# UT-Austin-RPL/FORGE

Hardware: AMD Instinct MI355X
Metric: rendered views/sec (5 views, 128^2 px, 64^3 voxel) (higher is better)
Workload: dtype f32; 1 GPU; BASELINE configs[1]: FORGE hot path, 1 scene(s)/GPU x 5 input views 256^2 -> 32^3x128 feature grid -> 64^3 render grid -> 5 views x 128^2 rays x 64 samples -> 5 RGB 256^2; HIP rotate, fp32-MFMA implicit-GEMM ResNet-50 trunk / conv1 / ConvGRU (Winograd F(2x2,3x3) x 3 depth taps) / heads / conv_rgb, HIP ray-march (no MIOpen/rocBLAS kernel in the step); eval BN, random-init seeded weights; scenes_per_gpu=1, views_in=5, views_out=5, feature_grid=32, render_grid=64, steps_in_flight=4, launch=hipGraph replay, 4 steps in flight on 4 HIP streams, parallelism=dp1 (scene-sharded, no data-path collective; 4-scalar RCC...

## Files before the change

forge_amd/_lib.py:

```python
import ctypes
import os

import torch

_HERE = os.path.dirname(os.path.abspath(__file__))
LIB_PATH = os.environ.get("FORGE_AMD_LIB") or os.path.join(_HERE, "libforge_hip.so")
_lib = None

_P = ctypes.c_void_p
_I = ctypes.c_int
_F = ctypes.c_float
_D = ctypes.c_double
_LL = ctypes.c_longlong

SIGNATURES = {
    "forge_version": [],
    "forge_last_error": [],
    "forge_rotate_fwd": [_P, _P, _P, _P, _I, _I, _I, _I, _I, _P],
    "forge_rotate_fwd_slots": [_P, _P, _P, _P, _P, _I, _I, _I, _I, _I, _P],
    "forge_rotate_xf_from_poses": [_P, _P, _P, _P, _P, _I, _I, _F, _P],
    "forge_rotate_bwd": [_P, _P, _P, _P, _P, _P, _I, _I, _I, _I, _I, _P],
    "forge_pose_chain_fwd": [_P, _P, _P, _P, _P, _F, _I, _I, _P, _P, _P, _P, _P, _P, _P, _P],
    "forge_colsum": [_P, _I, _P, _P, _LL, _I, _P],
    "forge_adam_small": [_P, _P, _P, _P, _P, _I, _F, _F, _F, _F, _P],
    "forge_rotate_bwd_slots": [_P, _P, _P, _P, _P, _P, _P, _I, _I, _I, _I, _I, _P],
    "forge_pose_chain_bwd": [_P, _P, _P, _P, _P, _I, _I, _P],
    "forge_pack_cameras": [_P, _LL, _LL, _LL, _P, _LL, _LL, _P, _LL, _LL, _LL, _P, _P, _I, _P],
    "forge_render_fwd": [_P, _P, _P, _P, _P, _P, _P] + [_I] * 9 + [_F] * 5 + [_P],
    "forge_render_bwd_ws_bytes": [_I] * 6,
    "forge_render_bwd": [_P, _P, _P, _P, _P, _P, _P, _P, _P, _P] + [_I] * 9 + [_F] * 5 + [_P, _LL, _P],
    "forge_resize_bilinear_fwd": [_P, _P, _I, _I, _I, _I, _I, _P],
    "forge_resize_bilinear_bwd": [_P, _P, _I, _I, _I, _I, _I, _P],
    "forge_conv_igemm": [_P, _I, _I, _LL, _P, _I, _I, _LL, _P, _P, _P, _P, _F, _P, _P, _P, _P, _P, _P] + [_I] * 10 + [_P] + [_I] * 12 + [_P, _LL, _P, _P],
    "forge_wino_weights": [_P, _P, _I, _I, _I, _I, _P],
    "forge_wino_dy": [_P, _I, _P, _I, _I, _I, _I, _I, _P],
    "forge_wino_wgrad": [_P, _P, _I, _LL, _LL, _P, _I, _LL, _LL, _P, _I, _I, _I, _I, _I, _I, _P],
    "forge_wino_dw": [_P, _P, _I, _I, _I, _P],
    "forge_wino_input": [_P, _I, _LL, _P, _I, _LL, _I, _I, _I, _I, _I, _I, _LL, _P],
    "forge_wino_input_dy": [_P, _I, _P, _P, _I, _I, _I, _I, _I, _P],
    "forge_wino_gemm": [_P, _I, _I, _LL, _LL, _P, _I, _I, _LL, _LL, _P, _P, _I, _I, _I, _I, _I, _I, _I, _P],
    "forge_wino_gemm_half": [_P, _I, _I, _LL, _LL, _P, _I, _I, _LL, _LL, _P, _P, _I, _I, _I, _I, _I, _I, _P],
    "forge_wino_gemm_dn": [_P, _I, _I, _LL, _LL, _P, _I, _I, _LL, _LL, _P, _P, _I, _I, _I, _I, _I, _I, _P],
    "forge_wino_weights_dn": [_P, _P, _I, _I, _P],
    "forge_wino_input_dn4": [_P, _I, _LL, _P, _I, _LL, _I, _I, _I, _I, _I, _I, _LL, _P],
    "forge_wino_weights_dn4": [_P, _P, _I, _I, _P],
    "forge_wino_gemm_dn4": [_P, _I, _I, _LL, _LL, _P, _I, _I, _LL, _LL, _P, _P, _I, _I, _I, _I, _I, _I, _P],
    "forge_wino_output_half": [_P, _P, _LL, _LL, _P, _P, _P, _F, _P, _P, _P, _P, _P, _P, _I, _I, _I, _I, _I, _I, _I, _P],
    "forge_wino_gemm_tile": [_LL, _I, _I],
    "forge_wino_output": [_P, _P, _LL, _LL, _P, _P, _P, _F, _P, _P, _P, _P, _P, _P, _I, _I, _I, _I, _I, _I, _I, _P],
    "forge_conv_igemm_plan": [_LL, _I, _I, _I, _I, _I, _I, _LL, _P, _P],
    "forge_conv_wgrad": [_P, _I, _P, _I, _I, _LL, _P, _I, _I, _LL, _P] + [_I] * 9 + [_P, _I, _P],
    "forge_conv_direct_fwd": [_P, _I, _P, _P, _F, _P, _I] + [_I] * 6 + [_P, _I, _P],
    "forge_conv_direct_dgrad": [_P, _I, _P, _P, _I] + [_I] * 6 + [_P, _I, _P],
    "forge_conv_direct_wgrad": [_P, _I, _P, _I, _P] + [_I] * 6 + [_P, _I, _P],
    "forge_gru_gates_fwd": [_P, _P, _P, _P, _P, _LL, _I, _P],
    "forge_gru_state_fwd": [_P, _P, _P, _P, _LL, _I, _P],
    "forge_gru_state_bwd": [_P, _I, _P, _P, _P, _P, _P, _P, _LL, _I, _P, _LL, _LL, _I, _P],
    "forge_gru_gates_bwd": [_P, _P, _I, _P, _P, _P, _P, _P, _P, _I, _LL, _I, _P, _LL, _LL, _I, _P],
    "forge_bn_ws_doubles": [_I],
    "forge_bn_train_fwd": [_P, _I, _P, _P, _F, _F, _P, _I, _P, _P, _P, _P, _F, _P, _LL, _I, _P, _I, _P, _I, _P],
    "forge_bn_train_bwd": [_P, _I, _P, _I, _P, _P, _P, _P, _F, _P, _I, _P, _P, _P, _LL, _I, _P, _I, _P, _I, _P],
    "forge_bn_sync_stats": [_P, _I, _P, _LL, _I, _I, _P],
    "forge_bn_eval_fwd": [_P, _I, _P, _P, _P, _P, _F, _F, _P, _I, _P, _P, _LL, _I, _P, _I, _P],
    "forge_bn_sync_fwd_apply": [_P, _I, _P, _P, _F, _F, _P, _I, _P, _P, _P, _P, _F, _P, _LL, _LL, _I, _P, _I, _P, _P],
    "forge_bn_sync_bwd_reduce": [_P, _I, _P, _I, _P, _P, _P, _P, _F, _P, _P, _P, _LL, _I, _P, _I, _P],
    "forge_bn_sync_bwd_apply": [_P, _I, _P, _I, _P, _P, _P, _P, _F, _P, _I, _P, _LL, _LL, _I, _P, _I, _P, _I, _P],
    "forge_affine_act_bwd": [_P, _I, _P, _I, _P, _F, _P, _I, _LL, _I, _P],
    "forge_sse_groups_blocks": [],
    "forge_sse_groups_fwd": [_P, _LL, _LL, _LL, _LL, _P, _P] + [_I] * 7 + [_P],
    "forge_sse_groups_bwd": [_P, _LL, _LL, _LL, _LL, _P, _P, _P] + [_I] * 7 + [_P],
    "forge_attention_fwd": [_P, _P, _P, _LL, _P, _I, _I, _I, _I, _P],
    "forge_attention_fwd_lse": [_P, _P, _P, _LL, _P, _P, _I, _I, _I, _I, _P],
    "forge_attention_bwd": [_P, _P, _P, _LL, _P, _P, _P, _P, _P, _P, _P, _I, _I, _I, _I, _P],
    "forge_attention_mh_fwd": [_P, _P, _P, _P, _P, _I, _I, _I, _I, _I] + [_LL] * 8 + [_F, _P],
    "forge_attention_mh_bwd": [_P] * 10 + [_I, _I, _I, _I, _I] + [_LL] * 8 + [_F, _P],
    "forge_token_linear_fwd": [_P, _LL, _P, _P, _P, _P, _F, _P, _LL, _P, _LL, _P, _P, _I, _I, _I, _I, _P],
    "forge_layer_norm_fwd": [_P, _LL, _P, _P, _F, _P, _LL, _P, _I, _I, _P],
    "forge_token_rows_plan": [_I, _I, _I, _P, _P],
    "forge_token_linear_bwd_ws_bytes": [_I, _I, _I, _I],
    "forge_token_linear_bwd": [_P, _LL, _P, _LL] + [_P] * 11 + [_LL, _I, _I, _I, _I, _P],
    "forge_layer_norm_bwd_ws_bytes": [_I, _I],
    "forge_layer_norm_bwd": [_P, _LL, _P, _LL] + [_P] * 6 + [_LL, _I, _I, _P],
    "forge_im2col_nchw": [_P, _P] + [_I] * 9 + [_P],
    "forge_maxpool2d_nhwc": [_P, _P] + [_I] * 7 + [_P],
    "forge_vgg_prep_fwd": [_P, _LL, _LL, _LL, _LL, _P, _LL, _LL, _LL, _LL, _P, _P, _P] + [_I] * 7 + [_P],
    "forge_vgg_prep_bwd": [_P, _I, _P, _P, _LL, _LL, _LL, _LL] + [_I] * 7 + [_P],
    "forge_l1_partial_blocks": [],
    "forge_l1_partial": [_P, _P, _LL, _P, _P],
    "forge_vgg_tap_bwd": [_P, _P, _P, _P, _P, _I, _I, _I, _I, _P],
    "forge_conv_wgrad_det": [_P, _I, _P, _I, _I, _LL, _P, _I, _I, _LL, _P] + [_I] * 9 + [_P, _I, _I, _P, _LL, _P],
    "forge_conv_wgrad_det_ws_bytes": [_I] * 11 + [_P, _I],
    "forge_conv_wgrad_plan": [_I] * 11 + [_P, _I, _I, _P],
    "forge_wino_wgrad_det": [_P, _P, _I, _LL, _LL, _P, _I, _LL, _LL, _P, _I, _I, _I, _I, _I, _I, _I, _P, _LL, _P],
    "forge_wino_wgrad_det_ws_bytes": [_I] * 8,
    "forge_conv_direct_wgrad_det": [_P, _I, _P, _I, _P] + [_I] * 6 + [_P, _I, _I, _P, _LL, _P],
    "forge_conv_direct_wgrad_det_ws_bytes": [_I] * 7,
    "forge_rotate_bwd_det": [_P, _P, _P, _P, _P, _P, _I, _I, _I, _I, _I, _I, _P, _LL, _P],
    "forge_rotate_bwd_det_ws_bytes": [_I] * 5,
    "forge_rotate_bwd_slots_det": [_P, _P, _P, _P, _P, _P, _P, _I, _I, _I, _I, _I, _I, _P, _LL, _P],
    "forge_rotate_bwd_slots_det_ws_bytes": [_I] * 5,
    "forge_metric_blocks": [],
    "forge_ssim_tiles": [_I, _I],
    "forge_psnr": [_P, _LL, _LL, _LL, _LL, _P, _LL, _LL, _LL, _LL, _I, _I, _I, _I, _D, _P, _P, _P],
    "forge_ssim": [_P, _LL, _LL, _LL, _LL, _P, _LL, _LL, _LL, _LL, _I, _I, _I, _I, _D, _P, _P, _P],
    "forge_lpips_tap": [_P, _I, _I, _I, _P, _P, _P],
    "forge_lpips_finalize": [_P, _I, _I, _I, _I, _I, _I, _P, _P],
    "forge_pose_sync": [_P, _P, _P, _I, _I, _I, _I, _I, _D, _P, _P, _P, _P],
    "forge_mesh_case_table": [_P, _I],
    "forge_mesh_workspace_bytes": [_I, _I, _I, _I],
    "forge_mesh_count": [_P, _I, _I, _I, _I, _F, _P, _LL, _P, _P],
    "forge_mesh_emit": [_P, _P, _I, _I, _I, _I, _I, _F, _F, _P, _LL, _P, _P, _I, _I, _P, _P, _P, _P, _P, _P],
    "forge_ncdhw_to_ndhwc": [_P, _P, _I, _I, _LL, _P],
    "forge_ndhwc_to_ncdhw": [_P, _P, _I, _I, _LL, _P],
}


_LL_RESULTS = ("forge_render_bwd_ws_bytes", "forge_conv_wgrad_det_ws_bytes", "forge_wino_wgrad_det_ws_bytes",
               "forge_conv_direct_wgrad_det_ws_bytes", "forge_rotate_bwd_det_ws_bytes", "forge_rotate_bwd_slots_det_ws_bytes",
               "forge_token_linear_bwd_ws_bytes", "forge_layer_norm_bwd_ws_bytes", "forge_mesh_workspace_bytes")


def lib():
    global _lib
    if _lib is None:
        if not os.path.exists(LIB_PATH):
            raise RuntimeError(
                "forge_amd: %s not found. Build it with `python -m forge_amd.build` (needs hipcc, "
                "targets gfx950). There is no CPU/PyTorch fallback for the HIP kernels." % LIB_PATH)
        h = ctypes.CDLL(LIB_PATH)
# ... 36 lines not shown
```

forge_amd/convops.py:

```python
import collections
import ctypes
import functools
import os
from fractions import Fraction

import torch

from . import _lib, determinism

EPI_BIAS, EPI_AFFINE_ACT, EPI_GRU_GATES, EPI_GRU_OUT = 0, 1, 2, 3


_TAPS_CACHE = {}


def _taps_array(taps):
    key = tuple(tuple(t) for t in taps)
    arr = _TAPS_CACHE.get(key)
    if arr is None:
        flat = [int(v) for t in key for v in t]
        arr = _TAPS_CACHE[key] = (ctypes.c_int * len(flat))(*flat)
    return arr


# ... 93 lines not shown
        return super().train(mode)

    def _apply(self, fn, *args, **kwargs):
        self.invalidate_packed()
        return super()._apply(fn, *args, **kwargs)


def invalidate_packed(module):
    for m in module.modules():
        if isinstance(m, PackedModule):
            m.invalidate_packed()


class _ZeroArena:

    def __init__(self):
        self.task, self.device = -1, None
        self.pools = {}
        self.want = {}

    def _end(self):
        self.want = {k: p[2] for k, p in self.pools.items()}
        self.pools, self.task = {}, -1

    HAVE_HOOKS = hasattr(torch._C, "_current_graph_task_id") and hasattr(getattr(torch.autograd.Variable, "_execution_engine", None), "queue_callback")

    def zeros(self, shape, device):
        n = 1
        for d in shape:
            n *= int(d)
        nbytes = (n * 4 + 255) // 256 * 256
        if not self.HAVE_HOOKS:
            return torch.zeros(shape, dtype=torch.float32, device=device)
        task = torch._C._current_graph_task_id()
        if task < 0:
            return torch.zeros(shape, dtype=torch.float32, device=device)
        if task != self.task:
            if self.task >= 0:
                self._end()
            self.task, self.device = task, device
            torch.autograd.Variable._execution_engine.queue_callback(self._end_of(task))
        if device != self.device:
            return torch.zeros(shape, dtype=torch.float32, device=device)
        key = torch.cuda.current_stream(device).cuda_stream if torch.device(device).type == "cuda" else 0
        pool = self.pools.get(key)
        if pool is None:
            want = self.want.get(key, 0)
            pool = self.pools[key] = [torch.zeros(want // 4 + 64, dtype=torch.float32, device=device) if want else None, 0, 0]
        pool[2] += nbytes
        if pool[0] is None or pool[1] + nbytes > pool[0].numel() * 4:
            return torch.zeros(shape, dtype=torch.float32, device=device)
        out = pool[0][pool[1] // 4:pool[1] // 4 + n].view(shape)
        pool[1] += nbytes
        return out

    def _end_of(self, task):
        def cb():
            if self.task == task:
                self._end()
        return cb


GRAD_ZEROS = _ZeroArena()


def grad_zeros(shape, device, scratch=False):
    if scratch:
        return torch.zeros(tuple(shape), dtype=torch.float32, device=device)
    return GRAD_ZEROS.zeros(tuple(shape), device)


SPLITK_WS_BYTES = 128 << 20

TILE_NAMES = {"A": "128, 128, 8, 1", "B": "64, 128, 8, 1", "C": "128, 64, 8, 1", "D": "64, 64, 4, 1", "E": "128, 32, 4, 1"}

_PLAN_CACHE = {}


class _State:
    plan_override = None
    winograd = True
    wino_depth_nest = os.environ.get("FORGE_WINO_DEPTH_NEST", "1") != "0"
    wino_depth_nest4 = os.environ.get("FORGE_WINO_DEPTH_NEST4", "1") != "0"


STATE = _State()


class force_plan:

    def __init__(self, tile=None, ksplit=None):
        self.val = (tile, ksplit)

    def __enter__(self):
        self.prev = STATE.plan_override
        STATE.plan_override = self.val
        return self

    def __exit__(self, *exc):
        STATE.plan_override = self.prev
        return False


def conv_plan(M, Cout, Cin, ntaps, epilogue, ldo, nphase=1):
    key = (int(M), int(Cout), int(Cin), int(ntaps), int(nphase), int(epilogue), int(ldo) % 4 == 0)
    pl = _PLAN_CACHE.get(key)
    if pl is None:
        tile, ks = ctypes.c_int(0), ctypes.c_int(0)
        _lib.check(_lib.lib().forge_conv_igemm_plan(int(M), int(Cout), int(Cin), int(ntaps), int(nphase), int(epilogue), int(ldo), SPLITK_WS_BYTES,
                                                    ctypes.byref(tile), ctypes.byref(ks)), "forge_conv_igemm_plan")
        pl = _PLAN_CACHE[key] = (chr(tile.value), ks.value)
    ov = STATE.plan_override
    if ov is not None and pl[0] != "N":
        tile = ov[0] or pl[0]
        ks = ov[1] if ov[1] is not None else (pl[1] if ov[0] is None else 1)
        can_split = nphase == 1 and epilogue in (EPI_BIAS, EPI_AFFINE_ACT) and Cout % 4 == 0 and ldo % 4 == 0
        if ks > 1 and not (can_split and ks * M * Cout * 4 <= SPLITK_WS_BYTES and ks <= (ntaps // nphase) * (Cin // 32)):
            ks = 1
        return tile, ks
    return pl


MAX_OPERAND_BYTES = (1 << 31) - 1


@_lib.on_tensor_device
def conv_igemm(in1, C1, ld1, in2, C2, ld2, wp, bias, scale, shift, slope, residual, aux_h, aux_z, out, out2,
               grid, in_grid, Cout, ldo, taps, out_grid=None, istride=1, ostride=1, phase=(0, 0, 0), epilogue=EPI_BIAS,
               bs1=0, bs2=0, lift=0, out3=None, stats=None):
    n, D, H, W = grid
    Di, Hi, Wi = in_grid
    Do, Ho, Wo = out_grid if out_grid is not None else (D, H, W)
    if wp.shape != (len(taps), Cout, C1 + C2):
        raise ValueError("packed weight %s does not match taps=%d Cout=%d Cin=%d" % (tuple(wp.shape), len(taps), Cout, C1 + C2))
    in_rows, out_rows = Di * Hi * Wi, Do * Ho * Wo
    b1, b2 = (int(bs1) or in_rows), (int(bs2) or in_rows)
    span = lambda k, br, ld: ((k - 1) * br + in_rows) * ld * 4
    limit = MAX_OPERAND_BYTES
    nc = n
    while nc > 1 and (span(nc, b1, ld1) > limit or (in2 is not None and span(nc, b2, ld2) > limit)):
        nc = (nc + 1) // 2
    L, st, arr = _lib.lib(), _lib.current_stream(), _taps_array(taps)
    nphase = 1
    if tuple(phase) == (-1, -1, -1):
        nphase = 8 if Do == 2 * D else 4

    def off(t, floats):
        return None if t is None else ctypes.c_void_p(t.data_ptr() + 4 * floats)
    gate_w = Cout // 2 if epilogue == EPI_GRU_GATES else Cout
    for s0 in range(0, n, nc):
        k = min(nc, n - s0)
        orow = s0 * out_rows
        tile, ksplit = conv_plan(k * D * H * W, Cout, C1 + C2, len(taps), epilogue, ldo, nphase)
        if stats is not None and (ksplit > 1 or nc < n):
            raise RuntimeError("forge_amd: conv_igemm output statistics need an un-chunked launch without split-K (use conv_stats_buffer)")
        ws = torch.empty(ksplit * k * D * H * W * Cout, dtype=torch.float32, device=out.device) if ksplit > 1 else None
        o_ld = gate_w if epilogue == EPI_GRU_GATES else ldo
        _lib.check(L.forge_conv_igemm(
            off(in1, s0 * b1 * ld1), C1, ld1, int(bs1), off(in2, s0 * b2 * ld2), C2, ld2, int(bs2), _lib.ptr(wp), _lib.ptr(bias), _lib.ptr(scale),
            _lib.ptr(shift), float(slope), off(residual, orow * (Cout if (lift or epilogue in (EPI_GRU_GATES, EPI_GRU_OUT)) else ldo)),
            off(aux_h, orow * gate_w), off(aux_z, orow * Cout),
            off(out, orow * (Cout if lift else o_ld)), off(out2, orow * o_ld), off(out3, orow * o_ld), k, D, H, W, istride, Di, Hi, Wi, Cout, ldo,
            arr, len(taps), ostride, phase[0], phase[1], phase[2], Do, Ho, Wo, epilogue, int(lift), 0 if tile == "N" else ord(tile), ksplit,
            _lib.ptr(ws), 0 if ws is None else ws.numel() * 4, _lib.ptr(stats), st),
            "forge_conv_igemm")
    return out
# ... 56 lines not shown
    return v


def conv3_launch(x1, C1, x2, C2, wp, bias, out, grid, Cout, bs1=0, residual=None, dgrad=False, U=None, wT=None):
    n, D, H, W = grid
    if wino_applies(TAPS_3x3x3, 1, n, D, H, W, C1, C2, Cout):
        return _wino_conv(x1, C1, bs1, x2, C2, 0, U if U is not None else wino_pack_packed(wp, transpose=dgrad), bias, out, residual, grid)
    w = (wT if wT is not None else wp.transpose(1, 2).contiguous()) if dgrad else wp
    taps = [(-a, -b, -c) for a, b, c in TAPS_3x3x3] if dgrad else TAPS_3x3x3
    if residual is None:
        return conv_igemm(x1, C1, C1, x2, C2, C2, w, bias, None, None, 1.0, None, None, None, out, None, grid, (D, H, W), Cout, Cout, taps,
                          epilogue=EPI_BIAS, bs1=bs1)
    one, zero = _one_zero(out.device, Cout)
    return conv_igemm(x1, C1, C1, x2, C2, C2, w, bias, one, zero, 1.0, residual, None, None, out, None, grid, (D, H, W), Cout, Cout, taps,
                      epilogue=EPI_AFFINE_ACT, bs1=bs1)


def wino_wgrad_applies(n, D, H, W, C1, C2, Cout, taps=None):
    return (wino_applies(TAPS_3x3x3 if taps is None else taps, 1, n, D, H, W, C1, C2, Cout) and C1 + C2 >= 128 and Cout >= 64 and (C2 == 0 or C1 % 128 == 0)
            and n * D * (H // 2) * (W // 2) * Cout * 4 <= MAX_OPERAND_BYTES)


@_lib.on_tensor_device
def conv3_wgrad(dy, x1, C1, x2, C2, dwp, grid, Cout, bs1=0, taps=None, dM=None):
    n, D, H, W = grid
    taps = TAPS_3x3x3 if taps is None else list(taps)
    if not wino_wgrad_applies(n, D, H, W, C1, C2, Cout, taps):
        return conv_wgrad(dy, x1, C1, x2, C2, dwp, grid, (D, H, W), Cout, taps, bs1=bs1)
    kd = len(taps) // 9
    L, st = _lib.lib(), _lib.current_stream()
    Ht, Wt = H // 2, W // 2
    R = n * D * Ht * Wt
    dev = dy.device
    V1 = wino_input(x1, C1, C1, n, D, H, W, bs=bs1)
    V2 = None if x2 is None else wino_input(x2, C2, C2, n, D, H, W)
    if dM is None:
        dM = torch.empty(16, R, Cout, dtype=torch.float32, device=dev)
        _lib.check(L.forge_wino_dy(_lib.ptr(dy), dy.shape[-1], _lib.ptr(dM), n, D, H, W, Cout, st), "forge_wino_dy")
    dU = grad_zeros((16, kd, Cout, C1 + C2), dev, scratch=True)
    determinism.launch("forge_wino_wgrad", (_lib.ptr(dM), _lib.ptr(V1), C1, 0, 0, _lib.ptr(V2), C2, 0, 0, _lib.ptr(dU), n, D, Ht, Wt, Cout, kd),
                       (C1, C2, n, D, Ht, Wt, Cout, kd), dev)
    _lib.check(L.forge_wino_dw(_lib.ptr(dU), _lib.ptr(dwp), Cout, C1 + C2, kd, st), "forge_wino_dw")
    return dwp


def wino_applies(taps, istride, n, D, H, W, C1, C2, Cout):
    tt = tuple(tuple(t) for t in taps)
    if not (wino_enabled() and istride == 1 and C1 % 32 == 0 and C2 % 32 == 0 and Cout % 8 == 0 and wino_fits(n, D, H, W, max(C1, C2, 1))):
        return False
    if len(tt) == 27 and tt == tuple(TAPS_3x3x3):
        return C1 + C2 >= 64 and Cout >= 32
    if len(tt) == 9 and tt == tuple(TAPS_3x3) and D == 1:
        return C2 == 0 and C1 >= WINO2D_MIN_C and Cout >= WINO2D_MIN_C
    return False


def wino_enabled():
    return STATE.winograd


class winograd:

    def __init__(self, on):
        self.on = bool(on)

    def __enter__(self):
        self.prev = STATE.winograd
        STATE.winograd = self.on
        return self

    def __exit__(self, *exc):
        STATE.winograd = self.prev
        return False


def wino_scene_chunk(b, D, H, W, C, views=1):
    nb = b
    while nb >= 1 and not wino_fits(nb, D, H, W, C, views=views):
        nb = (nb + 1) // 2 if nb > 1 else 0
    return nb


def wino_fits(n, D, H, W, C, views=1, nest4=False, form=None):
    rows = n * views * D * (H // 2) * (W // 2) * (form or WINO_FORMS["dn4" if nest4 else "points"]).rows
    return H % 2 == 0 and W % 2 == 0 and rows * C * 4 <= MAX_OPERAND_BYTES


@_lib.on_tensor_device
def wino_input_dy(dy, C, n, D, H, W):
    R = n * D * (H // 2) * (W // 2)
    V = torch.empty(16, R, C, dtype=torch.float32, device=dy.device)
    dM = torch.empty(16, R, C, dtype=torch.float32, device=dy.device)
    _lib.check(_lib.lib().forge_wino_input_dy(_lib.ptr(dy), C, _lib.ptr(V), _lib.ptr(dM), n, D, H, W, C, _lib.current_stream()), "forge_wino_input_dy")
    return V, dM


def wino_half_applies(R, Cout, Cin):
    return STATE.plan_override is None and wino_gemm_tile(R, Cout, Cin) == "B"


def wino_depth_nest_applies(R, D, Ht, Wt, Cout, Cin):
    return (STATE.wino_depth_nest and STATE.plan_override is None and D % 2 == 0 and (Ht * Wt) % 64 == 0 and Cin % 32 == 0
            and R * Cout * 4 <= MAX_OPERAND_BYTES and wino_gemm_tile(R, Cout, Cin) == "B")


def wino_depth_nest4_applies(R, D, Ht, Wt, Cout, Cin):
    return STATE.wino_depth_nest4 and D % 4 == 0 and D >= 8 and wino_depth_nest_applies(R, D, Ht, Wt, Cout, Cin)


WinoForm = collections.namedtuple("WinoForm", "name P gemm weights ushape input rows kloops applies tile metered")
_U4 = lambda kd, co_, ci_: (16, kd, co_, ci_)
WINO_FORMS = {f.name: f for f in (
    WinoForm("points", 16, "forge_wino_gemm", "forge_wino_weights", _U4, "forge_wino_input", 1, None, lambda R, D, Ht, Wt, Cout, Cin: True,
             True, True),
    WinoForm("half", 8, "forge_wino_gemm_half", "forge_wino_weights", _U4, "forge_wino_input", 1, None,
             lambda R, D, Ht, Wt, Cout, Cin: wino_half_applies(R, Cout, Cin), False, True),
    WinoForm("dn", 16, "forge_wino_gemm_dn", "forge_wino_weights_dn", lambda kd, co_, ci_: (16, 2, 2, co_, ci_), "forge_wino_input", 1, 2,
             lambda *a: wino_depth_nest_applies(*a), False, True),
    WinoForm("dn4", 16, "forge_wino_gemm_dn4", "forge_wino_weights_dn4", lambda kd, co_, ci_: (16, 6, co_, ci_), "forge_wino_input_dn4", Fraction(3, 2),
             Fraction(3, 2), lambda *a: wino_depth_nest4_applies(*a), False, False),
)}


def wino_calls(form):
    if not form.metered:
        return functools.partial(wino_form_input, form), functools.partial(wino_form_gemm, form)
    return (lambda *a, **kw: wino_input(*a, **kw)), (lambda *a, **kw: wino_gemm(*a, **kw))


@_lib.on_tensor_device
def wino_pack(form, wp, transpose=False):
    T, co_, ci_ = wp.shape
    nest = form.kloops is not None
    assert T == 27 or (T == 9 and not nest)
    assert not (nest and transpose)
    kd = T // 9
    wp = wp.detach()
    wp = wp if wp.is_contiguous() else wp.contiguous()
    U = torch.empty(form.ushape(kd, ci_, co_) if transpose else form.ushape(kd, co_, ci_), dtype=torch.float32, device=wp.device)
    own = () if nest else (kd, 1 if transpose else 0)
    _lib.check(getattr(_lib.lib(), form.weights)(_lib.ptr(wp), _lib.ptr(U), co_, ci_, *own, _lib.current_stream()), form.weights)
    return U


@_lib.on_tensor_device
def wino_form_input(form, x, C, ld, n, D, H, W, bs=0, out=None, nsum=1, sum_stride=0):
    rows = int(n * D * (H // 2) * (W // 2) * form.rows)
    V = out if out is not None else torch.empty(16, rows, C, dtype=torch.float32, device=x.device)
    if form.rows != 1 and (V.shape != (16, rows, C) or not V.is_contiguous()):
        raise ValueError("depth-nest operand buffer %s is not [16][%d][%d]" % (tuple(V.shape), rows, C))
    _lib.check(getattr(_lib.lib(), form.input)(_lib.ptr(x), ld, int(bs), _lib.ptr(V), C, 0, n, D, H, W, C, int(nsum), int(sum_stride), _lib.current_stream()),
               form.input)
    return V


def wino_input(x, C, ld, n, D, H, W, bs=0, out=None, nsum=1, sum_stride=0):
    return wino_form_input(WINO_FORMS["points"], x, C, ld, n, D, H, W, bs=bs, out=out, nsum=nsum, sum_stride=sum_stride)


def _point_products(Mm, P, R, Cout, device):
    if Mm is None:
        Mm = torch.empty(P, R, Cout, dtype=torch.float32, device=device)
    if not (Mm.is_contiguous() and Mm.dtype == torch.float32 and Mm.numel() >= P * R * Cout):
        raise ValueError("point-product buffer %s %s%s cannot hold %d x %d x %d float32" % (
            tuple(Mm.shape), Mm.dtype, "" if Mm.is_contiguous() else " (not contiguous)", P, R, Cout))
    if Mm.shape != (P, R, Cout):
        Mm = Mm.as_strided((P, R, Cout), (R * Cout, Cout, 1))
    return Mm


@_lib.on_tensor_device
def wino_form_gemm(form, V1, C1, V2, C2, U, Mm, n, D, Ht, Wt, Cout, view=0, views=1):
    R = n * D * Ht * Wt
    vol = int(D * Ht * Wt * form.rows)
    nest = form.kloops is not None
    kd = 3 if nest else U.shape[1]
    if U.shape != form.ushape(kd, Cout, C1 + C2) or (kd not in (1, 3)) or (nest and not U.is_contiguous()):
        raise ValueError("%s weight %s does not match Cout=%d Cin=%d" % ("depth-nest" if nest else "transformed", tuple(U.shape), Cout, C1 + C2))
    if form.rows != 1 and (V1.shape[1] != n * views * vol or (V2 is not None and V2.shape[1] != n * vol)):
        raise ValueError("depth-nest operands %s / %s are not %s's %d (x %d views) rows per point" % (
            tuple(V1.shape), None if V2 is None else tuple(V2.shape), form.input, n * vol, views))
    Mm = _point_products(Mm, form.P, R, Cout, V1.device)
    tile = (ord(wino_gemm_tile(R, Cout, C1 + C2)),) if form.tile else ()
    p1 = ctypes.c_void_p(V1.data_ptr() + 4 * view * vol * C1)
    _lib.check(getattr(_lib.lib(), form.gemm)(p1, C1, C1, views * vol if views > 1 else 0, V1.shape[1] * C1, _lib.ptr(V2), C2, C2, 0,
                                              0 if V2 is None else V2.shape[1] * C2, _lib.ptr(U), _lib.ptr(Mm), n, D, Ht, Wt, Cout, kd,
                                              *tile, _lib.current_stream()), form.gemm)
    return Mm


def wino_gemm(V1, C1, V2, C2, U, Mm, n, D, Ht, Wt, Cout, view=0, views=1, half=None):
    if U.dim() == 5:
        form = "dn"
    else:
        if half is None:
            half = WINO_FORMS["half"].applies(n * D * Ht * Wt, D, Ht, Wt, Cout, C1 + C2)
        form = "half" if half else "points"
    return wino_form_gemm(WINO_FORMS[form], V1, C1, V2, C2, U, Mm, n, D, Ht, Wt, Cout, view=view, views=views)


def wino_gemm_tile(R, Cout, Cin):
    ov = STATE.plan_override
    if ov is not None and ov[0]:
        return ov[0]
    return chr(_lib.lib().forge_wino_gemm_tile(int(R), int(Cout), int(Cin)))


@_lib.on_tensor_device
def wino_output(Mm, bias, scale, shift, slope, residual, aux_h, aux_z, out, out2, out3, n, D, H, W, Cout, ldo, epilogue, Mm2=None, view=0, views=1):
    vol = D * (H // 2) * (W // 2)
    P = Mm.shape[0] if Mm.dim() == 3 else 0
    if P not in (8, 16) or Mm.shape[1:] != (n * vol, Cout) or not Mm.is_contiguous():
        raise ValueError("point products %s do not match [8 | 16][%d][%d]" % (tuple(Mm.shape), n * vol, Cout))
    if Mm2 is not None and (Mm2.shape != (P, n * views * vol, Cout) or not Mm2.is_contiguous()):
        raise ValueError("second addend %s does not match [%d][%d][%d] (the form of Mm)" % (tuple(Mm2.shape), P, n * views * vol, Cout))
    p2 = None if Mm2 is None else ctypes.c_void_p(Mm2.data_ptr() + 4 * view * vol * Cout)
    fn, name = (_lib.lib().forge_wino_output_half, "forge_wino_output_half") if P == 8 else (_lib.lib().forge_wino_output, "forge_wino_output")
    _lib.check(fn(_lib.ptr(Mm), p2, views * vol, 0 if Mm2 is None else Mm2.shape[1] * Cout, _lib.ptr(bias), _lib.ptr(scale), _lib.ptr(shift), float(slope),
                  _lib.ptr(residual), _lib.ptr(aux_h), _lib.ptr(aux_z), _lib.ptr(out), _lib.ptr(out2), _lib.ptr(out3), n, D, H, W, Cout, ldo, epilogue,
                  _lib.current_stream()), name)
    return out


@_lib.on_tensor_device
def conv_wgrad(dy, x1, C1, x2, C2, dwp, grid, in_grid, Cout, taps, istride=1, bs1=0, bs2=0):
    if x2 is not None and C1 % 128:
        x1 = torch.cat([x1[..., :C1], x2[..., :C2]], dim=-1)
        C1, x2, C2, bs1, bs2 = C1 + C2, None, 0, 0, 0
    n, D, H, W = grid
    Di, Hi, Wi = in_grid
    in_rows, out_rows = Di * Hi * Wi, D * H * W
    ldy, ld1, ld2 = dy.shape[-1], x1.shape[-1], (0 if x2 is None else x2.shape[-1])
    b1, b2 = (int(bs1) or in_rows), (int(bs2) or in_rows)
    span = lambda k, br, ld, rows: ((k - 1) * br + rows) * ld * 4
    nc = n
    while nc > 1 and (span(nc, out_rows, ldy, out_rows) > MAX_OPERAND_BYTES or span(nc, b1, ld1, in_rows) > MAX_OPERAND_BYTES
                      or (x2 is not None and span(nc, b2, ld2, in_rows) > MAX_OPERAND_BYTES)):
        nc = (nc + 1) // 2
    off = lambda t, floats: None if t is None else ctypes.c_void_p(t.data_ptr() + 4 * floats)
    ta = _taps_array(taps)
    for s0 in range(0, n, nc):
        k = min(nc, n - s0)
        determinism.launch("forge_conv_wgrad", (off(dy, s0 * out_rows * ldy), ldy, off(x1, s0 * b1 * ld1), C1, ld1, int(bs1), off(x2, s0 * b2 * ld2), C2, ld2,
                                                int(bs2), _lib.ptr(dwp), k, D, H, W, istride, Di, Hi, Wi, Cout, ta, len(taps)),
                           (C1, C2, k, D, H, W, istride, Di, Hi, Wi, Cout, ta, len(taps)), dwp.device)
    return dwp


def _batch_stride_rows(x):
    n, D, H, W, C = x.shape
    if x.stride()[1:] != (H * W * C, W * C, C, 1):
        raise ValueError("conv_rows needs channels-last rows [n,D,H,W,C] dense within a batch element; got strides %s" % (x.stride(),))
    return 0 if (n == 1 or x.stride(0) == D * H * W * C) else x.stride(0) // C


@_lib.on_tensor_device
def colsum(x):
    C = x.shape[-1]
    rows = x.reshape(-1, C)
    if not (rows.is_cuda and rows.dtype == torch.float32):
        raise RuntimeError("forge_amd: colsum runs only on the MI355X HIP kernels (float32 cuda tensor); got %s on %s" % (rows.dtype, rows.device))
    if C % 4:
        if C > 32:
            raise RuntimeError("forge_amd: colsum needs C %% 4 == 0 or C <= 32 (got %d)" % C)
        rows = rows if rows.is_contiguous() else rows.contiguous()
    else:
        rows = rows if (rows.stride(1) == 1 and rows.stride(0) >= C and rows.stride(0) % 4 == 0) else rows.contiguous()
    out = torch.empty(C, dtype=torch.float32, device=rows.device)
    ws = torch.empty(_lib.lib().forge_bn_ws_doubles(C), dtype=torch.float64, device=rows.device)
    _lib.check(_lib.lib().forge_colsum(_lib.ptr(rows), rows.stride(0), _lib.ptr(out), _lib.ptr(ws), rows.shape[0], C, _lib.current_stream()), "forge_colsum")
    return out


class _ConvTapsRows(torch.autograd.Function):

    @staticmethod
    def forward(ctx, x1, x2, wp, bias, taps, istride, out_spatial, want_stats=False):
        n, Di, Hi, Wi, C1 = x1.shape
        C2 = 0 if x2 is None else x2.shape[-1]
        T, Cout, Cin = wp.shape
        D, H, W = out_spatial
        wpc = wp.detach().contiguous()
        out = torch.empty(n, D, H, W, Cout, dtype=torch.float32, device=x1.device)
        bs1 = _batch_stride_rows(x1)
        bs2 = 0 if x2 is None else _batch_stride_rows(x2)
        stats = None
        if (D, H, W) == (Di, Hi, Wi) and wino_applies(taps, istride, n, D, H, W, C1, C2, Cout):
            wino_conv_rows(x1, x2, wino_pack_packed(wpc), bias, out)
        else:
            if want_stats and bs1 == 0 and bs2 == 0:
                stats = conv_stats_buffer(x1, x2, (n, D, H, W), (Di, Hi, Wi), Cout, Cin, T, Cout, x1.device)
            conv_igemm(x1, C1, C1, x2, C2, C2, wpc, bias, None, None, 1.0, None, None, None, out, None,
                       (n, D, H, W), (Di, Hi, Wi), Cout, Cout, taps, istride=istride, epilogue=EPI_BIAS, bs1=bs1, bs2=bs2, stats=stats)
        ctx.save_for_backward(x1, x2, wpc)
        ctx.meta = (tuple(taps), istride, (D, H, W), bias is not None)
        if not want_stats:
# ... 308 lines not shown
```

forge_amd/csrc/conv_igemm.hip:

```cpp
#include "common.h"
#include <cmath>
#include <type_traits>

namespace forge {

enum ConvEpilogue : int {
    EPI_BIAS = 0,
    EPI_AFFINE_ACT = 1,
    EPI_GRU_GATES = 2,
    EPI_GRU_OUT = 3,
};

constexpr int MAX_TAPS = 64;

struct ConvArgs {
    const float* in1; const float* in2;
    int C1, C2, ld1, ld2;
    long long bs1r, bs2r;
    long long span1, span2;
    const float* wp;
    const float* bias;
    const float* scale; const float* shift; float slope;
    const float* aux_h; const float* aux_z;
    float* out; float* out2; float* out3;
// ... 1033 lines not shown
                  "forge_conv_igemm: row strides must cover the channels and keep 16-byte alignment");
    ConvArgs a;
    a.in1 = in1; a.in2 = in2; a.C1 = C1; a.C2 = C2; a.ld1 = ld1; a.ld2 = ld2;
    a.bs1r = bs1 > 0 ? bs1 : (long long)Di * Hi * Wi; a.bs2r = bs2 > 0 ? bs2 : (long long)Di * Hi * Wi;
    a.span1 = ((long long)(n - 1) * a.bs1r + (long long)Di * Hi * Wi) * ld1 * 4;
    a.span2 = in2 ? ((long long)(n - 1) * a.bs2r + (long long)Di * Hi * Wi) * ld2 * 4 : 0;
    FORGE_REQUIRE(a.span1 < (1ll << 31) && a.span2 < (1ll << 31) && (long long)ntaps * Cout * (C1 + C2) * 4 < (1ll << 31), FORGE_ESHAPE,
                  "forge_conv_igemm: an operand spans >= 2 GiB (32-bit buffer offsets); split the batch");
    a.is = is; a.Di = Di; a.Hi = Hi; a.Wi = Wi; a.residual = residual;
    a.ldr = (lift > 0 || epilogue == EPI_GRU_GATES || epilogue == EPI_GRU_OUT) ? Cout : ldo;
    a.lift = lift; a.ws = nullptr; a.ksplit = 1; a.stats = stats;
    a.wp = wp; a.bias = bias; a.scale = scale; a.shift = shift; a.slope = slope;
    a.aux_h = aux_h; a.aux_z = aux_z; a.out = out; a.out2 = out2; a.out3 = out3; a.n = n; a.D = D; a.H = H; a.W = W; a.Cout = Cout; a.ldo = ldo;
    a.ntaps = ntaps; a.os = os; a.pz = pz; a.py = py; a.px = px; a.Do = Do; a.Ho = Ho; a.Wo = Wo; a.epi = epilogue;
    a.nphase = 1; a.tpp = ntaps; a.nbat = 1; a.pt1 = a.pt2 = a.ptw = a.pto = 0;
    if (pz < 0) {
        FORGE_REQUIRE(os == 2 && py < 0 && px < 0 && Ho == 2 * H && Wo == 2 * W && (Do == 2 * D || Do == D), FORGE_EINVAL,
                      "forge_conv_igemm: merged phases (pz = py = px = -1) need os = 2 and a doubled output grid");
        a.nphase = Do == 2 * D ? 8 : 4;
        FORGE_REQUIRE(ntaps % a.nphase == 0, FORGE_EINVAL, "forge_conv_igemm: merged phases need ntaps %% %d == 0", a.nphase);
        a.tpp = ntaps / a.nphase;
        a.pz = a.py = a.px = 0;
    }
    for (int k = 0; k < 3 * ntaps; ++k)
        FORGE_REQUIRE(taps[k] >= -128 && taps[k] <= 127, FORGE_EINVAL, "forge_conv_igemm: tap %d component %d = %d outside [-128, 127]", k / 3, k % 3, taps[k]);
    for (int t = 0; t < MAX_TAPS; ++t) {
        for (int k = 0; k < 3; ++k) a.tap[t][k] = (signed char)(t < ntaps ? taps[t * 3 + k] : 0);
        a.tap[t][3] = 0;
    }
    const long long M = (long long)n * D * H * W;
    FORGE_REQUIRE(M < (1ll << 31), FORGE_ESHAPE, "forge_conv_igemm: more than 2^31 GEMM rows; split the batch");
    FORGE_REQUIRE(out3 == nullptr || epilogue == EPI_GRU_GATES || epilogue == EPI_GRU_OUT, FORGE_EINVAL, "forge_conv_igemm: out3 is a GRU-epilogue output");
    hipStream_t st = (hipStream_t)stream;
    if (Cout <= 16) {
        FORGE_REQUIRE(epilogue == EPI_BIAS || epilogue == EPI_AFFINE_ACT, FORGE_EINVAL, "forge_conv_igemm: GRU epilogues need Cout > 16");
        const long long grid = (M + BM16 - 1) / BM16 * a.nphase;
        FORGE_REQUIRE(grid < (1ll << 31), FORGE_ESHAPE, "forge_conv_igemm: grid too large");
        int lines_r = 0;
        if (a.nphase == 1 && is == 1 && os == 1 && lift == 0 && Do == D && Ho == H && Wo == W && Di == D && Hi == H && Wi == W && pz == 0 && py == 0 && px == 0) {
            for (int r = 1; r <= 2 && !lines_r; ++r) {
                const int nt = 2 * r + 1;
                bool ok = ntaps % nt == 0 && W > r;
                for (int t = 0; ok && t < ntaps; ++t)
                    ok = taps[t * 3 + 2] == (t % nt) - r && taps[t * 3] == taps[(t - t % nt) * 3] && taps[t * 3 + 1] == taps[(t - t % nt) * 3 + 1];
                if (ok) lines_r = r;
            }
        }
        if (lines_r == 1) hipLaunchKernelGGL(conv_igemm_n16_lines_kernel<1>, dim3((unsigned)grid), dim3(NTHREADS), 0, st, a);
        else if (lines_r == 2) hipLaunchKernelGGL(conv_igemm_n16_lines_kernel<2>, dim3((unsigned)grid), dim3(NTHREADS), 0, st, a);
        else hipLaunchKernelGGL(conv_igemm_n16_kernel, dim3((unsigned)grid), dim3(NTHREADS), 0, st, a);
    } else {
        const bool can_split = a.nphase == 1 && splitk_ws && (epilogue == EPI_BIAS || epilogue == EPI_AFFINE_ACT) && Cout % 4 == 0 && ldo % 4 == 0;
        ConvPlan pl;
        if (tile == 0) {
            pl = plan_conv(M * a.nphase, Cout, C1 + C2, a.tpp, can_split, splitk_ws_bytes);
        } else {
            pl = ConvPlan{(char)tile, ksplit > 1 ? ksplit : 1};
            FORGE_REQUIRE(tile >= 'A' && tile <= 'E', FORGE_EINVAL, "forge_conv_igemm: tile '%c' is not one of A..E (0 = planned here)", (char)tile);
            FORGE_REQUIRE(pl.ksplit == 1 || (can_split && pl.ksplit <= 8 && (long long)pl.ksplit * M * Cout * 4 <= splitk_ws_bytes &&
                                             pl.ksplit <= a.tpp * ((C1 + C2) / BK)), FORGE_EINVAL,
                          "forge_conv_igemm: ksplit=%d needs epilogue 0/1 without phases, Cout, ldo %% 4 == 0 and a workspace of ksplit M Cout floats", pl.ksplit);
        }
        FORGE_REQUIRE(stats == nullptr || (tile != 0 && pl.ksplit == 1), FORGE_EINVAL,
                      "forge_conv_igemm: output statistics need an explicit tile ('A'..'E' from forge_conv_igemm_plan) and a plan without split-K");
        if (pl.ksplit > 1) { a.ksplit = pl.ksplit; a.ws = splitk_ws; }
        if (int rc = launch_conv_tile(a, pl.tile, st)) return rc;
        if (a.ksplit > 1) {
            const long long total = M * (Cout / 4);
            hipLaunchKernelGGL(conv_splitk_epilogue_kernel, dim3((unsigned)((total + 255) / 256)), dim3(256), 0, st, a);
        }
    }
    FORGE_LAUNCH_CHECK("forge_conv_igemm");
    return 0;
}

extern "C" int forge_wino_gemm_tile(long long R, int Cout, int Cin) {
    (void)Cin;
    if (Cout <= 64) return R < 2048 ? 'D' : 'C';
    return R < 2048 ? 'D' : 'B';
}

static int wino_gemm_impl(const float* V1, int C1, int ld1, long long bs1, long long pt1, const float* V2, int C2, int ld2, long long bs2,
                          long long pt2, const float* U, float* Mm, int n, int D, int Ht, int Wt, int Cout, int kd, int tile, int form, forge_stream_t stream) {
    const bool half = form == 1, dn = form == 2, dn4 = form == 3;
    FORGE_REQUIRE(tile == 0 || (tile >= 'A' && tile <= 'E'), FORGE_EINVAL, "forge_wino_gemm: tile must be 0 (default rule) or 'A'..'E'");
    FORGE_REQUIRE(V1 && U && Mm && (kd == 1 || kd == 3), FORGE_EINVAL, "forge_wino_gemm: null pointer argument / kd not 1 or 3");
    FORGE_REQUIRE(n > 0 && D > 0 && Ht > 0 && Wt > 0 && Cout > 16, FORGE_EINVAL, "forge_wino_gemm: bad dims n=%d D=%d Ht=%d Wt=%d Cout=%d (Cout > 16)", n,
                  D, Ht, Wt, Cout);
    FORGE_REQUIRE(C1 > 0 && C1 % BK == 0 && C2 >= 0 && C2 % BK == 0 && (C2 == 0) == (V2 == nullptr), FORGE_ESHAPE,
                  "forge_wino_gemm: C1=%d / C2=%d must be multiples of %d, V2 given iff C2 > 0", C1, C2, BK);
    FORGE_REQUIRE(ld1 >= C1 && ld1 % 4 == 0 && (C2 == 0 || (ld2 >= C2 && ld2 % 4 == 0)), FORGE_EINVAL, "forge_wino_gemm: bad row strides");
    FORGE_REQUIRE(!dn || (kd == 3 && D % 2 == 0 && ((long long)Ht * Wt) % 64 == 0), FORGE_EINVAL,
                  "forge_wino_gemm_dn: needs three depth taps, an even D and Ht Wt %% 64 == 0 (kd=%d D=%d Ht=%d Wt=%d)", kd, D, Ht, Wt);
    FORGE_REQUIRE(!dn4 || (kd == 3 && D % 4 == 0 && ((long long)Ht * Wt) % 64 == 0), FORGE_EINVAL,
                  "forge_wino_gemm_dn4: needs three depth taps, D %% 4 == 0 and Ht Wt %% 64 == 0 (kd=%d D=%d Ht=%d Wt=%d)", kd, D, Ht, Wt);
    ConvArgs a;
    memset(&a, 0, sizeof(a));
    const long long vol = (long long)D * Ht * Wt, R = (long long)n * vol, rows = dn4 ? vol / 4 * 6 : vol, Cin = C1 + C2;
    const int npos = dn4 ? 6 : dn ? 4 : kd;
    a.in1 = V1; a.in2 = V2; a.C1 = C1; a.C2 = C2; a.ld1 = ld1; a.ld2 = ld2; a.bs1r = bs1 > 0 ? bs1 : rows; a.bs2r = bs2 > 0 ? bs2 : rows;
    a.span1 = ((long long)(n - 1) * a.bs1r + rows) * ld1 * 4;
    a.span2 = V2 ? ((long long)(n - 1) * a.bs2r + rows) * ld2 * 4 : 0;
    if (dn4) {
        FORGE_REQUIRE(a.span1 < (1ll << 31) && a.span2 < (1ll << 31) && R * Cout * 4 < (1ll << 31) && 6ll * Cout * Cin * 4 < (1ll << 31), FORGE_EINVAL,
                      "forge_wino_gemm_dn4: an operand or an output plane spans >= 2 GiB (32-bit buffer offsets); split the batch");
    } else {
        FORGE_REQUIRE(a.span1 < (1ll << 31) && a.span2 < (1ll << 31) && R < (1ll << 31), FORGE_ESHAPE,
                      "forge_wino_gemm: an operand spans >= 2 GiB per Winograd point (32-bit buffer offsets); split the batch");
        FORGE_REQUIRE(!dn || (R * Cout * 4 < (1ll << 31) && 4ll * Cout * Cin * 4 < (1ll << 31)), FORGE_ESHAPE,
                      "forge_wino_gemm_dn: an output plane spans >= 2 GiB (32-bit buffer offsets); split the batch");
    }
    a.wp = U; a.slope = 1.f; a.out = Mm; a.n = n; a.D = D; a.H = Ht; a.W = Wt; a.is = 1; a.Di = D; a.Hi = Ht; a.Wi = Wt;
    a.Cout = Cout; a.ldo = Cout; a.ldr = Cout; a.ntaps = a.tpp = npos; a.os = 1; a.Do = D; a.Ho = Ht; a.Wo = Wt; a.nphase = 1; a.epi = EPI_BIAS;
    a.ksplit = 1; a.nbat = half ? 4 : 16;
    a.pt1 = pt1 > 0 ? pt1 : (long long)n * rows * ld1; a.pt2 = V2 ? (pt2 > 0 ? pt2 : (long long)n * rows * ld2) : 0;
    a.ptw = (long long)npos * Cout * Cin; a.pto = R * Cout;
    if (form == 0 || half) {
        if (kd == 3) { a.tap[0][0] = -1; a.tap[2][0] = 1; }
        if (!tile) tile = forge_wino_gemm_tile(R, Cout, C1 + C2);
    }
    if (int rc = launch_conv_tile(a, (char)tile, (hipStream_t)stream, form)) return rc;
    FORGE_LAUNCH_CHECK(dn4 ? "forge_wino_gemm_dn4" : dn ? "forge_wino_gemm_dn" : "forge_wino_gemm");
    return 0;
}

extern "C" int forge_wino_gemm(const float* V1, int C1, int ld1, long long bs1, long long pt1, const float* V2, int C2, int ld2, long long bs2,
                               long long pt2, const float* U, float* Mm, int n, int D, int Ht, int Wt, int Cout, int kd, int tile, forge_stream_t stream) {
    return wino_gemm_impl(V1, C1, ld1, bs1, pt1, V2, C2, ld2, bs2, pt2, U, Mm, n, D, Ht, Wt, Cout, kd, tile, 0, stream);
}

extern "C" int forge_wino_gemm_half(const float* V1, int C1, int ld1, long long bs1, long long pt1, const float* V2, int C2, int ld2, long long bs2,
                                    long long pt2, const float* U, float* Mm8, int n, int D, int Ht, int Wt, int Cout, int kd, forge_stream_t stream) {
    return wino_gemm_impl(V1, C1, ld1, bs1, pt1, V2, C2, ld2, bs2, pt2, U, Mm8, n, D, Ht, Wt, Cout, kd, 'B', 1, stream);
}

extern "C" int forge_wino_gemm_dn(const float* V1, int C1, int ld1, long long bs1, long long pt1, const float* V2, int C2, int ld2, long long bs2,
                                  long long pt2, const float* Ud, float* Mm, int n, int D, int Ht, int Wt, int Cout, int kd, forge_stream_t stream) {
    FORGE_REQUIRE(C1 > 0 && C1 % BK == 0 && C2 >= 0 && C2 % BK == 0, FORGE_EINVAL, "forge_wino_gemm_dn: C1=%d / C2=%d must be multiples of %d", C1, C2, BK);
    return wino_gemm_impl(V1, C1, ld1, bs1, pt1, V2, C2, ld2, bs2, pt2, Ud, Mm, n, D, Ht, Wt, Cout, kd, 'B', 2, stream);
}

extern "C" int forge_wino_gemm_dn4(const float* V1, int C1, int ld1, long long bs1, long long pt1, const float* V2, int C2, int ld2, long long bs2,
                                   long long pt2, const float* Ud, float* Mm, int n, int D, int Ht, int Wt, int Cout, int kd, forge_stream_t stream) {
    FORGE_REQUIRE(C1 > 0 && C1 % BK == 0 && C2 >= 0 && C2 % BK == 0, FORGE_EINVAL, "forge_wino_gemm_dn4: C1=%d / C2=%d must be multiples of %d", C1, C2, BK);
    return wino_gemm_impl(V1, C1, ld1, bs1, pt1, V2, C2, ld2, bs2, pt2, Ud, Mm, n, D, Ht, Wt, Cout, kd, 'B', 3, stream);
}
```

forge_amd/csrc/winograd.hip:

```cpp
#include "common.h"

namespace forge {

__device__ __forceinline__ float4 add(float4 a, float4 b) { return make_float4(a.x + b.x, a.y + b.y, a.z + b.z, a.w + b.w); }
__device__ __forceinline__ float4 sub(float4 a, float4 b) { return make_float4(a.x - b.x, a.y - b.y, a.z - b.z, a.w - b.w); }
__device__ __forceinline__ float add(float a, float b) { return a + b; }
__device__ __forceinline__ float sub(float a, float b) { return a - b; }

__device__ __forceinline__ void tile_decode(long long idx, int per, int cs, int Ht, int Wt, unsigned& r, int& c, int& tw, int& th, unsigned& t) {
    r = (unsigned)(idx / per);
    c = (int)(idx - (long long)r * per) << cs;
    unsigned q = r;
    t = q / (unsigned)Wt;
    tw = (int)(q - t * (unsigned)Wt); q = t; t = q / (unsigned)Ht;
    th = (int)(q - t * (unsigned)Ht);
}

template <typename T, typename I>
__device__ __forceinline__ void bt_d_b_store(const T (&d)[4][4], float* V, I row, int ld, int c, long long ptv) {
    T w[4][4];
#pragma unroll
    for (int j = 0; j < 4; ++j) {
        w[0][j] = sub(d[0][j], d[2][j]);
        w[1][j] = add(d[1][j], d[2][j]);
        w[2][j] = sub(d[2][j], d[1][j]);
        w[3][j] = sub(d[1][j], d[3][j]);
    }
    float* vp = V + (long long)row * ld + c;
#pragma unroll
    for (int i = 0; i < 4; ++i) {
        *reinterpret_cast<T*>(vp + (4 * i + 0) * ptv) = sub(w[i][0], w[i][2]);
        *reinterpret_cast<T*>(vp + (4 * i + 1) * ptv) = add(w[i][1], w[i][2]);
        *reinterpret_cast<T*>(vp + (4 * i + 2) * ptv) = sub(w[i][2], w[i][1]);
        *reinterpret_cast<T*>(vp + (4 * i + 3) * ptv) = sub(w[i][1], w[i][3]);
    }
}

__device__ __forceinline__ void a_y_at_store(float4 y00, float4 y01, float4 y10, float4 y11, float* mp, long long ptm) {
    const float4 zero = make_float4(0.f, 0.f, 0.f, 0.f);
    const float4 s[4][2] = {{y00, y01}, {add(y00, y10), add(y01, y11)}, {sub(y00, y10), sub(y01, y11)}, {sub(zero, y10), sub(zero, y11)}};
#pragma unroll
    for (int i = 0; i < 4; ++i) {
        *reinterpret_cast<float4*>(mp + (4 * i + 0) * ptm) = s[i][0];
        *reinterpret_cast<float4*>(mp + (4 * i + 1) * ptm) = add(s[i][0], s[i][1]);
        *reinterpret_cast<float4*>(mp + (4 * i + 2) * ptm) = sub(s[i][0], s[i][1]);
        *reinterpret_cast<float4*>(mp + (4 * i + 3) * ptm) = sub(zero, s[i][1]);
    }
}

__device__ __forceinline__ void g_d_gt_store(const double (&d)[3][3], float* up, long long pt) {
    double g[4][3];
#pragma unroll
    for (int b = 0; b < 3; ++b) {
        g[0][b] = d[0][b];
        g[1][b] = 0.5 * (d[0][b] + d[1][b] + d[2][b]);
        g[2][b] = 0.5 * (d[0][b] - d[1][b] + d[2][b]);
        g[3][b] = d[2][b];
    }
#pragma unroll
    for (int i = 0; i < 4; ++i) {
        up[(4 * i + 0) * pt] = (float)g[i][0];
        up[(4 * i + 1) * pt] = (float)(0.5 * (g[i][0] + g[i][1] + g[i][2]));
        up[(4 * i + 2) * pt] = (float)(0.5 * (g[i][0] - g[i][1] + g[i][2]));
        up[(4 * i + 3) * pt] = (float)g[i][2];
    }
}

struct WinoInArgs {
    const float* in; int ld; long long bs;
    float* V; int ldv; long long ptv;
    int n, D, H, W, C;
    int nsum; long long ss;
    float* dM; long long ptm;
};

template <bool DY>
__global__ __launch_bounds__(256) void wino_input_kernel(const WinoInArgs a) {
    const int C4 = a.C >> 2, Ht = a.H >> 1, Wt = a.W >> 1;
    const long long idx = (long long)xcd_remap(blockIdx.x, gridDim.x) * 256 + threadIdx.x;
    const long long R = (long long)a.n * a.D * Ht * Wt;
    if (idx >= R * C4) return;
    unsigned r, t;
    int c, tw, th;
    tile_decode(idx, C4, 2, Ht, Wt, r, c, tw, th, t);
    const unsigned q = t; t = q / (unsigned)a.D;
    const int z = (int)(q - t * (unsigned)a.D);
    const float* base = a.in + ((long long)t * a.bs + (long long)z * a.H * a.W) * a.ld + c;
    float4 d[4][4];
#pragma unroll
    for (int i = 0; i < 4; ++i) {
        const int y = 2 * th - 1 + i;
#pragma unroll
        for (int j = 0; j < 4; ++j) {
            const int x = 2 * tw - 1 + j;
            const bool ok = (unsigned)y < (unsigned)a.H && (unsigned)x < (unsigned)a.W;
            float4 v = make_float4(0.f, 0.f, 0.f, 0.f);
            if (ok) {
                const float* p = base + ((long long)y * a.W + x) * a.ld;
                v = *reinterpret_cast<const float4*>(p);
                if (a.nsum > 1) {
                    for (int k = 1; k < a.nsum; ++k) v = add(v, *reinterpret_cast<const float4*>(p + (long long)k * a.ss * a.ld));
                    const float inv = 1.f / (float)a.nsum;
                    v = make_float4(v.x * inv, v.y * inv, v.z * inv, v.w * inv);
                }
            }
            d[i][j] = v;
        }
    }
    if constexpr (DY) a_y_at_store(d[1][1], d[1][2], d[2][1], d[2][2], a.dM + (long long)r * a.C + c, a.ptm);
    bt_d_b_store(d, a.V, r, a.ldv, c, a.ptv);
}

__global__ __launch_bounds__(256) void wino_input_dn4_kernel(const WinoInArgs a) {
    const int Ht = a.H >> 1, Wt = a.W >> 1, Dg = a.D >> 2;
    const long long idx = (long long)xcd_remap(blockIdx.x, gridDim.x) * 256 + threadIdx.x;
    const long long RG = (long long)a.n * Dg * Ht * Wt;
    if (idx >= RG * a.C) return;
    unsigned r, t;
    int c, tw, th;
    tile_decode(idx, a.C, 0, Ht, Wt, r, c, tw, th, t);
    const unsigned q = t; t = q / (unsigned)Dg;
    const int g = (int)(q - t * (unsigned)Dg);
    const long long HW = (long long)a.H * a.W;
    const float* base = a.in + (long long)t * a.bs * a.ld + c;
    const float inv = 1.f / (float)a.nsum;
    float d[6][4][4];
#pragma unroll
    for (int i = 0; i < 4; ++i) {
        const int y = 2 * th - 1 + i;
#pragma unroll
        for (int j = 0; j < 4; ++j) {
            const int x = 2 * tw - 1 + j;
            const bool ok = (unsigned)y < (unsigned)a.H && (unsigned)x < (unsigned)a.W;
            float p[6];
#pragma unroll
            for (int e = 0; e < 6; ++e) {
                const int z = 4 * g - 1 + e;
                float v = 0.f;
                if (ok && (unsigned)z < (unsigned)a.D) {
                    const float* s = base + ((long long)z * HW + (long long)y * a.W + x) * a.ld;
                    v = *s;
                    if (a.nsum > 1) {
                        for (int k = 1; k < a.nsum; ++k) v += s[(long long)k * a.ss * a.ld];
                        v *= inv;
                    }
                }
                p[e] = v;
            }
            const float a02 = p[0] - p[2], a24 = p[2] - p[4], s34 = p[3] + p[4], s12 = p[1] + p[2], d43 = p[4] - p[3], d12 = p[1] - p[2];
            const float d42 = p[4] - p[2], d31 = p[3] - p[1], d13 = p[1] - p[3], d35 = p[3] - p[5];
            d[0][i][j] = fmaf(4.f, a02, -a24);
            d[1][i][j] = fmaf(-4.f, s12, s34);
            d[2][i][j] = fmaf(4.f, d12, d43);
            d[3][i][j] = fmaf(2.f, d31, d42);
            d[4][i][j] = fmaf(-2.f, d31, d42);
            d[5][i][j] = fmaf(4.f, d13, -d35);
        }
    }
    const long long HWt = (long long)Ht * Wt;
    float* vp = a.V + ((((long long)t * Dg + g) * 6) * HWt + (long long)th * Wt + tw) * a.ldv + c;
#pragma unroll
    for (int k = 0; k < 6; ++k) bt_d_b_store(d[k], vp, k * HWt, a.ldv, 0, a.ptv);
}

__global__ __launch_bounds__(256) void wino_weight_kernel(const float* __restrict__ wp, float* __restrict__ U, int Cout, int Cin, int KD, int transpose) {
    const int No = transpose ? Cin : Cout, Nc = transpose ? Cout : Cin;
    const long long idx = (long long)blockIdx.x * 256 + threadIdx.x, per = (long long)No * Nc;
    if (idx >= KD * per) return;
    const int kd = (int)(idx / per);
    const long long oc = idx - kd * per;
    const int o = (int)(oc / Nc), c = (int)(oc - (long long)o * Nc);
    double w[3][3];
#pragma unroll
    for (int a = 0; a < 3; ++a)
#pragma unroll
        for (int b = 0; b < 3; ++b) {
            const int tap = transpose ? ((KD - 1 - kd) * 3 + (2 - a)) * 3 + (2 - b) : (kd * 3 + a) * 3 + b;
            w[a][b] = (double)wp[((long long)tap * Cout + (transpose ? c : o)) * Cin + (transpose ? o : c)];
        }
    g_d_gt_store(w, U + ((long long)kd * No + o) * Nc + c, KD * per);
}

__device__ __forceinline__ double depth_row_f23(int k, double w0, double w1, double w2) {
    return k == 0 ? w0 : k == 1 ? 0.5 * (w0 + w1 + w2) : k == 2 ? 0.5 * (w0 - w1 + w2) : w2;
}
__device__ __forceinline__ double depth_row_f43(int k, double w0, double w1, double w2) {
    return k == 0 ? 0.25 * w0 : k == 1 ? -((w0 + w2) + w1) / 6.0 : k == 2 ? -((w0 + w2) - w1) / 6.0
         : k == 3 ? ((0.25 * w0 + w2) + 0.5 * w1) / 6.0 : k == 4 ? ((0.25 * w0 + w2) - 0.5 * w1) / 6.0 : w2;
}

template <int K, double (*ROW)(int, double, double, double)>
__global__ __launch_bounds__(256) void wino_weight_nest_kernel(const float* __restrict__ wp, float* __restrict__ U, int Cout, int Cin) {
    const long long idx = (long long)blockIdx.x * 256 + threadIdx.x, per = (long long)Cout * Cin;
    if (idx >= per) return;
    double w[3][3][3];
#pragma unroll
    for (int t = 0; t < 27; ++t) w[t / 9][(t / 3) % 3][t % 3] = (double)wp[t * per + idx];
#pragma unroll
    for (int k = 0; k < K; ++k) {
        double d[3][3];
#pragma unroll
        for (int a = 0; a < 3; ++a)
#pragma unroll
            for (int b = 0; b < 3; ++b) d[a][b] = ROW(k, w[0][a][b], w[1][a][b], w[2][a][b]);
        g_d_gt_store(d, U + k * per + idx, K * per);
    }
}

enum WinoEpilogue : int { W_BIAS = 0, W_AFFINE_ACT = 1, W_GRU_GATES = 2, W_GRU_OUT = 3 };

struct WinoOutArgs {
    const float* Mm; long long ptm;
    const float* Mm2; long long ptm2, bs2;
    const float* bias; const float* scale; const float* shift; float slope;
    const float* residual;
    const float* aux_h; const float* aux_z;
    float* out; float* out2; float* out3; int ldo;
    int n, D, H, W, Cout, epi;
};

template <int ROWS>
__device__ __forceinline__ void load_planes(float4 (&m)[ROWS][4], const float* Mm, long long ptm, const float* Mm2, long long ptm2, long long bs2, int Cout, unsigned R1, unsigned r, int c) {
    const float* mp = Mm + (long long)r * Cout + c;
#pragma unroll
    for (int i = 0; i < ROWS; ++i)
#pragma unroll
        for (int j = 0; j < 4; ++j) m[i][j] = *reinterpret_cast<const float4*>(mp + (4 * i + j) * ptm);
    if (Mm2) {
        const unsigned nn = r / R1;
        const float* mp2 = Mm2 + ((long long)nn * bs2 + (r - nn * R1)) * Cout + c;
#pragma unroll
        for (int i = 0; i < ROWS; ++i)
#pragma unroll
            for (int j = 0; j < 4; ++j) m[i][j] = add(m[i][j], *reinterpret_cast<const float4*>(mp2 + (4 * i + j) * ptm2));
    }
}

template <int EPI, bool HALF = false>
__global__ __launch_bounds__(256) void wino_output_kernel(const WinoOutArgs a) {
    const int C4 = a.Cout >> 2, Ht = a.H >> 1, Wt = a.W >> 1;
    const long long idx = (long long)blockIdx.x * 256 + threadIdx.x;
    const long long R = (long long)a.n * a.D * Ht * Wt;
    if (idx >= R * C4) return;
    unsigned r, t;
    int c, tw, th;
    tile_decode(idx, C4, 2, Ht, Wt, r, c, tw, th, t);
    float4 s[2][4];
    if constexpr (HALF) {
        load_planes<2>(s, a.Mm, a.ptm, a.Mm2, a.ptm2, a.bs2, a.Cout, (unsigned)(a.D * Ht * Wt), r, c);
    } else {
        float4 m[4][4];
        load_planes<4>(m, a.Mm, a.ptm, a.Mm2, a.ptm2, a.bs2, a.Cout, (unsigned)(a.D * Ht * Wt), r, c);
#pragma unroll
        for (int j = 0; j < 4; ++j) {
            s[0][j] = add(add(m[0][j], m[1][j]), m[2][j]);
            s[1][j] = sub(sub(m[1][j], m[2][j]), m[3][j]);
        }
    }
    float4 y[2][2];
#pragma unroll
    for (int i = 0; i < 2; ++i) {
        y[i][0] = add(add(s[i][0], s[i][1]), s[i][2]);
        y[i][1] = sub(sub(s[i][1], s[i][2]), s[i][3]);
    }
    float4 bias = make_float4(0.f, 0.f, 0.f, 0.f), sc = make_float4(1.f, 1.f, 1.f, 1.f), sh = bias;
    if (a.bias) bias = *reinterpret_cast<const float4*>(a.bias + c);
    if ((EPI == W_AFFINE_ACT || (EPI == W_GRU_OUT && a.out2)) && a.scale) {
        sc = *reinterpret_cast<const float4*>(a.scale + c);
        sh = *reinterpret_cast<const float4*>(a.shift + c);
    }
    const int Ch = a.Cout >> 1;
    const long long plane = (long long)t * a.H * a.W;
#pragma unroll
    for (int i = 0; i < 2; ++i)
#pragma unroll
        for (int j = 0; j < 2; ++j) {
            const long long orow = plane + (long long)(2 * th + i) * a.W + (2 * tw + j);
            float v[4] = {y[i][j].x + bias.x, y[i][j].y + bias.y, y[i][j].z + bias.z, y[i][j].w + bias.w};
            if (a.residual) {
                const float4 rr = *reinterpret_cast<const float4*>(a.residual + orow * a.Cout + c);
                v[0] += rr.x; v[1] += rr.y; v[2] += rr.z; v[3] += rr.w;
            }
            const float scv[4] = {sc.x, sc.y, sc.z, sc.w}, shv[4] = {sh.x, sh.y, sh.z, sh.w};
            if constexpr (EPI == W_BIAS) {
                *reinterpret_cast<float4*>(a.out + orow * a.ldo + c) = make_float4(v[0], v[1], v[2], v[3]);
            } else if constexpr (EPI == W_AFFINE_ACT) {
#pragma unroll
                for (int k = 0; k < 4; ++k) {
                    const float u = fmaf(v[k], scv[k], shv[k]);
                    v[k] = u > 0.f ? u : u * a.slope;
                }
                *reinterpret_cast<float4*>(a.out + orow * a.ldo + c) = make_float4(v[0], v[1], v[2], v[3]);
            } else if constexpr (EPI == W_GRU_GATES) {
                float g[4];
#pragma unroll
                for (int k = 0; k < 4; ++k) g[k] = 1.f / (1.f + expf(-v[k]));
                if (c < Ch) {
                    *reinterpret_cast<float4*>(a.out + orow * Ch + c) = make_float4(g[0], g[1], g[2], g[3]);
                } else {
                    const float4 h = *reinterpret_cast<const float4*>(a.aux_h + orow * Ch + (c - Ch));
                    *reinterpret_cast<float4*>(a.out2 + orow * Ch + (c - Ch)) = make_float4(h.x * g[0], h.y * g[1], h.z * g[2], h.w * g[3]);
                    if (a.out3) *reinterpret_cast<float4*>(a.out3 + orow * Ch + (c - Ch)) = make_float4(g[0], g[1], g[2], g[3]);
                }
            } else {
                const float4 z4 = *reinterpret_cast<const float4*>(a.aux_z + orow * a.Cout + c);
                const float4 h4 = *reinterpret_cast<const float4*>(a.aux_h + orow * a.Cout + c);
                const float zv[4] = {z4.x, z4.y, z4.z, z4.w}, hv[4] = {h4.x, h4.y, h4.z, h4.w};
                float cand[4], hn[4];
#pragma unroll
                for (int k = 0; k < 4; ++k) {
                    cand[k] = tanhf(v[k]);
                    hn[k] = hv[k] * (1.f - zv[k]) + cand[k] * zv[k];
                }
                *reinterpret_cast<float4*>(a.out + orow * a.ldo + c) = make_float4(hn[0], hn[1], hn[2], hn[3]);
                if (a.out2)
                    *reinterpret_cast<float4*>(a.out2 + orow * a.ldo + c) =
                        make_float4(fmaf(hn[0], scv[0], shv[0]), fmaf(hn[1], scv[1], shv[1]), fmaf(hn[2], scv[2], shv[2]), fmaf(hn[3], scv[3], shv[3]));
                if (a.out3) *reinterpret_cast<float4*>(a.out3 + orow * a.ldo + c) = make_float4(cand[0], cand[1], cand[2], cand[3]);
            }
        }
}

struct WinoDyArgs {
    const float* dy; int ldy;
    float* dM; long long ptm;
    int n, D, H, W, Cout;
};

__global__ __launch_bounds__(256) void wino_dy_kernel(const WinoDyArgs a) {
    const int C4 = a.Cout >> 2, Ht = a.H >> 1, Wt = a.W >> 1;
    const long long idx = (long long)blockIdx.x * 256 + threadIdx.x;
    const long long R = (long long)a.n * a.D * Ht * Wt;
    if (idx >= R * C4) return;
    unsigned r, t;
    int c, tw, th;
    tile_decode(idx, C4, 2, Ht, Wt, r, c, tw, th, t);
    const float* yp = a.dy + ((long long)t * a.H * a.W + (long long)(2 * th) * a.W + 2 * tw) * a.ldy + c;
    float4 y[2][2];
#pragma unroll
    for (int i = 0; i < 2; ++i)
#pragma unroll
        for (int j = 0; j < 2; ++j) y[i][j] = *reinterpret_cast<const float4*>(yp + ((long long)i * a.W + j) * a.ldy);
    a_y_at_store(y[0][0], y[0][1], y[1][0], y[1][1], a.dM + (long long)r * a.Cout + c, a.ptm);
}

__global__ __launch_bounds__(256) void wino_dw_kernel(const float* __restrict__ dU, float* __restrict__ dw, int Cout, int Cin, int KD) {
    const long long idx = (long long)blockIdx.x * 256 + threadIdx.x, per = (long long)Cout * Cin;
    if (idx >= KD * per) return;
    const int kd = (int)(idx / per);
    const long long oc = idx - kd * per;
    const long long pt = KD * per;
    float u[4][4];
#pragma unroll
    for (int i = 0; i < 4; ++i)
#pragma unroll
        for (int j = 0; j < 4; ++j) u[i][j] = dU[(4 * i + j) * pt + kd * per + oc];
    float g[3][4];
#pragma unroll
    for (int j = 0; j < 4; ++j) {
        g[0][j] = u[0][j] + 0.5f * (u[1][j] + u[2][j]);
        g[1][j] = 0.5f * (u[1][j] - u[2][j]);
        g[2][j] = 0.5f * (u[1][j] + u[2][j]) + u[3][j];
    }
#pragma unroll
    for (int a_ = 0; a_ < 3; ++a_) {
        float* o = dw + ((long long)((kd * 3 + a_) * 3) * per) + oc;
        o[0 * per] += g[a_][0] + 0.5f * (g[a_][1] + g[a_][2]);
        o[1 * per] += 0.5f * (g[a_][1] - g[a_][2]);
        o[2 * per] += 0.5f * (g[a_][1] + g[a_][2]) + g[a_][3];
    }
}

}

using namespace forge;

extern "C" int forge_wino_dy(const float* dy, int ldy, float* dM, int n, int D, int H, int W, int Cout, forge_stream_t stream) {
    FORGE_REQUIRE(dy && dM, FORGE_EINVAL, "forge_wino_dy: null pointer argument");
    FORGE_REQUIRE(n > 0 && D > 0 && H > 0 && W > 0 && H % 2 == 0 && W % 2 == 0 && Cout > 0 && Cout % 4 == 0 && ldy >= Cout && ldy % 4 == 0, FORGE_ESHAPE,
                  "forge_wino_dy: n=%d D=%d H=%d W=%d Cout=%d ldy=%d (H, W even; Cout, ldy multiples of 4)", n, D, H, W, Cout, ldy);
    WinoDyArgs a;
    const long long R = (long long)n * D * (H / 2) * (W / 2);
    a.dy = dy; a.ldy = ldy; a.dM = dM; a.ptm = R * Cout; a.n = n; a.D = D; a.H = H; a.W = W; a.Cout = Cout;
    FORGE_REQUIRE(R < (1ll << 31), FORGE_ESHAPE, "forge_wino_dy: more than 2^31 tiles; split the batch");
    const long long total = R * (Cout / 4), grid = (total + 255) / 256;
    FORGE_REQUIRE(grid < (1ll << 31), FORGE_ESHAPE, "forge_wino_dy: grid too large");
    hipLaunchKernelGGL(wino_dy_kernel, dim3((unsigned)grid), dim3(256), 0, (hipStream_t)stream, a);
    FORGE_LAUNCH_CHECK("forge_wino_dy");
    return 0;
}

extern "C" int forge_wino_dw(const float* dU, float* dw, int Cout, int Cin, int kd, forge_stream_t stream) {
    FORGE_REQUIRE(dU && dw && Cout > 0 && Cin > 0 && (kd == 1 || kd == 3), FORGE_EINVAL, "forge_wino_dw: bad argument (kd = 1 or 3)");
    const long long total = (long long)kd * Cout * Cin;
    hipLaunchKernelGGL(wino_dw_kernel, dim3((unsigned)((total + 255) / 256)), dim3(256), 0, (hipStream_t)stream, dU, dw, Cout, Cin, kd);
    FORGE_LAUNCH_CHECK("forge_wino_dw");
    return 0;
}

template <typename K, typename... A>
static int wino_weights_launch(const char* name, K kernel, long long total, forge_stream_t stream, A... args) {
    hipLaunchKernelGGL(kernel, dim3((unsigned)((total + 255) / 256)), dim3(256), 0, (hipStream_t)stream, args...);
    FORGE_LAUNCH_CHECK(name);
    return 0;
}

extern "C" int forge_wino_weights(const float* wp, float* U, int Cout, int Cin, int kd, int transpose, forge_stream_t stream) {
    FORGE_REQUIRE(wp && U && Cout > 0 && Cin > 0 && (kd == 1 || kd == 3), FORGE_EINVAL, "forge_wino_weights: bad argument (kd = 1 or 3)");
    return wino_weights_launch("forge_wino_weights", wino_weight_kernel, (long long)kd * Cout * Cin, stream, wp, U, Cout, Cin, kd, transpose);
}

extern "C" int forge_wino_weights_dn(const float* wp, float* Ud, int Cout, int Cin, forge_stream_t stream) {
    FORGE_REQUIRE(wp && Ud && Cout > 0 && Cin > 0, FORGE_EINVAL, "forge_wino_weights_dn: bad argument");
    return wino_weights_launch("forge_wino_weights_dn", wino_weight_nest_kernel<4, depth_row_f23>, (long long)Cout * Cin, stream, wp, Ud, Cout, Cin);
}

extern "C" int forge_wino_weights_dn4(const float* wp, float* Ud, int Cout, int Cin, forge_stream_t stream) {
    FORGE_REQUIRE(wp && Ud && Cout > 0 && Cin > 0, FORGE_EINVAL, "forge_wino_weights_dn4: bad argument");
    return wino_weights_launch("forge_wino_weights_dn4", wino_weight_nest_kernel<6, depth_row_f43>, (long long)Cout * Cin, stream, wp, Ud, Cout, Cin);
}

enum WinoInKind { IN_PLAIN, IN_DN4, IN_DY };

static int wino_input_impl(const char* name, WinoInKind kind, const float* in, int ld, long long bs, float* V, int ldv, long long ptv, float* dM, int n, int D, int H,
                           int W, int C, int nsum, long long sum_stride, forge_stream_t stream) {
    const bool dn4 = kind == IN_DN4;
    FORGE_REQUIRE(in && V && (kind != IN_DY || dM), FORGE_EINVAL, "%s: null pointer argument", name);
    FORGE_REQUIRE(nsum >= 1 && (nsum == 1 || sum_stride > 0), FORGE_EINVAL, "%s: nsum >= 1, and a positive sum_stride (rows) with nsum > 1", name);
    FORGE_REQUIRE(!dn4 || (D > 0 && D % 4 == 0), FORGE_EINVAL, "%s: D=%d must be a multiple of 4", name, D);
    const bool ok = n > 0 && D > 0 && H > 0 && W > 0 && H % 2 == 0 && W % 2 == 0 && C > 0 && C % 4 == 0 && ld >= C && ld % 4 == 0 && ldv >= C && ldv % 4 == 0;
    if (kind == IN_DY)
        FORGE_REQUIRE(ok, FORGE_ESHAPE, "%s: n=%d D=%d H=%d W=%d C=%d ld=%d (H, W even; C, ld multiples of 4)", name, n, D, H, W, C, ld);
    FORGE_REQUIRE(ok, FORGE_ESHAPE, "%s: n=%d D=%d H=%d W=%d C=%d ld=%d ldv=%d (H, W even; C, ld, ldv multiples of 4)", name, n, D, H, W, C, ld, ldv);
    WinoInArgs a;
    a.in = in; a.ld = ld; a.bs = bs > 0 ? bs : (long long)D * H * W; a.V = V; a.ldv = ldv; a.n = n; a.D = D; a.H = H; a.W = W; a.C = C;
    a.nsum = nsum; a.ss = sum_stride;
    const long long R = (long long)n * (dn4 ? D / 4 : D) * (H / 2) * (W / 2), rows = dn4 ? 6 * R : R;
    a.ptv = ptv > 0 ? ptv : rows * ldv;
    a.dM = dM; a.ptm = dM ? R * C : 0;
    FORGE_REQUIRE(rows < (1ll << 31), FORGE_ESHAPE, dn4 ? "%s: more than 2^31 operand rows; split the batch" : "%s: more than 2^31 tiles; split the batch", name);
    const long long total = R * (dn4 ? C : C / 4), grid = (total + 255) / 256;
    FORGE_REQUIRE(grid < (1ll << 31), FORGE_ESHAPE, "%s: grid too large", name);
    const dim3 g((unsigned)grid), b(256);
    if (dn4) hipLaunchKernelGGL(wino_input_dn4_kernel, g, b, 0, (hipStream_t)stream, a);
    else if (kind == IN_DY) hipLaunchKernelGGL(wino_input_kernel<true>, g, b, 0, (hipStream_t)stream, a);
    else hipLaunchKernelGGL(wino_input_kernel<false>, g, b, 0, (hipStream_t)stream, a);
    FORGE_LAUNCH_CHECK(name);
    return 0;
}

extern "C" int forge_wino_input(const float* in, int ld, long long bs, float* V, int ldv, long long ptv, int n, int D, int H, int W, int C,
                                int nsum, long long sum_stride, forge_stream_t stream) {
    return wino_input_impl("forge_wino_input", IN_PLAIN, in, ld, bs, V, ldv, ptv, nullptr, n, D, H, W, C, nsum, sum_stride, stream);
}

extern "C" int forge_wino_input_dn4(const float* in, int ld, long long bs, float* V6, int ldv, long long ptv, int n, int D, int H, int W, int C,
                                    int nsum, long long sum_stride, forge_stream_t stream) {
    return wino_input_impl("forge_wino_input_dn4", IN_DN4, in, ld, bs, V6, ldv, ptv, nullptr, n, D, H, W, C, nsum, sum_stride, stream);
}

extern "C" int forge_wino_input_dy(const float* dy, int ld, float* V, float* dM, int n, int D, int H, int W, int C, forge_stream_t stream) {
    return wino_input_impl("forge_wino_input_dy", IN_DY, dy, ld, 0, V, C, 0, dM, n, D, H, W, C, 1, 0, stream);
}

static int wino_output_impl(const float* Mm, const float* Mm2, long long bs2, long long pt2, const float* bias, const float* scale, const float* shift, float slope, const float* residual,
                            const float* aux_h, const float* aux_z, float* out, float* out2, float* out3, int n, int D, int H, int W, int Cout,
                            int ldo, int epilogue, bool half, forge_stream_t stream) {
    FORGE_REQUIRE(Mm && out, FORGE_EINVAL, "forge_wino_output: null pointer argument");
    FORGE_REQUIRE(n > 0 && D > 0 && H > 0 && W > 0 && H % 2 == 0 && W % 2 == 0 && Cout > 0 && Cout % 8 == 0 && ldo % 4 == 0, FORGE_ESHAPE,
                  "forge_wino_output: n=%d D=%d H=%d W=%d Cout=%d ldo=%d (H, W even; Cout multiple of 8; ldo of 4)", n, D, H, W, Cout, ldo);
    FORGE_REQUIRE(epilogue >= 0 && epilogue <= 3, FORGE_EINVAL, "forge_wino_output: unknown epilogue %d", epilogue);
    FORGE_REQUIRE(epilogue == W_GRU_GATES ? ldo == Cout / 2 : ldo >= Cout, FORGE_ESHAPE,
                  "forge_wino_output: ldo=%d (epilogues 0, 1, 3: ldo >= Cout=%d; epilogue 2: ldo == Cout / 2)", ldo, Cout);
    FORGE_REQUIRE(epilogue != W_AFFINE_ACT || (scale && shift), FORGE_EINVAL, "forge_wino_output: affine epilogue needs scale/shift");
    FORGE_REQUIRE(epilogue != W_GRU_GATES || (aux_h && out2), FORGE_EINVAL, "forge_wino_output: GRU gate epilogue needs aux_h, out2");
    FORGE_REQUIRE(epilogue != W_GRU_OUT || (aux_h && aux_z && (!out2 || (scale && shift))), FORGE_EINVAL,
                  "forge_wino_output: GRU out epilogue needs aux_h, aux_z (and scale/shift with out2)");
    FORGE_REQUIRE(out3 == nullptr || epilogue == W_GRU_GATES || epilogue == W_GRU_OUT, FORGE_EINVAL, "forge_wino_output: out3 is a GRU-epilogue output");
    WinoOutArgs a;
    const long long R = (long long)n * D * (H / 2) * (W / 2);
    a.Mm = Mm; a.ptm = R * Cout; a.Mm2 = Mm2; a.bs2 = bs2 > 0 ? bs2 : (long long)D * (H / 2) * (W / 2); a.ptm2 = pt2 > 0 ? pt2 : R * Cout; a.bias = bias; a.scale = scale; a.shift = shift; a.slope = slope; a.residual = residual; a.aux_h = aux_h; a.aux_z = aux_z;
    a.out = out; a.out2 = out2; a.out3 = out3; a.ldo = ldo; a.n = n; a.D = D; a.H = H; a.W = W; a.Cout = Cout; a.epi = epilogue;
    FORGE_REQUIRE(R < (1ll << 31), FORGE_ESHAPE, "forge_wino_output: more than 2^31 tiles; split the batch");
    const long long total = R * (Cout / 4), grid = (total + 255) / 256;
    FORGE_REQUIRE(grid < (1ll << 31), FORGE_ESHAPE, "forge_wino_output: grid too large");
    const dim3 g((unsigned)grid), b(256);
    hipStream_t st = (hipStream_t)stream;
    if (half) {
        switch (epilogue) {
            case W_BIAS: hipLaunchKernelGGL((wino_output_kernel<W_BIAS, true>), g, b, 0, st, a); break;
            case W_AFFINE_ACT: hipLaunchKernelGGL((wino_output_kernel<W_AFFINE_ACT, true>), g, b, 0, st, a); break;
            case W_GRU_GATES: hipLaunchKernelGGL((wino_output_kernel<W_GRU_GATES, true>), g, b, 0, st, a); break;
            default: hipLaunchKernelGGL((wino_output_kernel<W_GRU_OUT, true>), g, b, 0, st, a); break;
        }
    } else {
        switch (epilogue) {
            case W_BIAS: hipLaunchKernelGGL(wino_output_kernel<W_BIAS>, g, b, 0, st, a); break;
            case W_AFFINE_ACT: hipLaunchKernelGGL(wino_output_kernel<W_AFFINE_ACT>, g, b, 0, st, a); break;
            case W_GRU_GATES: hipLaunchKernelGGL(wino_output_kernel<W_GRU_GATES>, g, b, 0, st, a); break;
            default: hipLaunchKernelGGL(wino_output_kernel<W_GRU_OUT>, g, b, 0, st, a); break;
        }
    }
    FORGE_LAUNCH_CHECK("forge_wino_output");
    return 0;
}

extern "C" int forge_wino_output(const float* Mm, const float* Mm2, long long bs2, long long pt2, const float* bias, const float* scale, const float* shift, float slope, const float* residual,
                                 const float* aux_h, const float* aux_z, float* out, float* out2, float* out3, int n, int D, int H, int W, int Cout,
                                 int ldo, int epilogue, forge_stream_t stream) {
    return wino_output_impl(Mm, Mm2, bs2, pt2, bias, scale, shift, slope, residual, aux_h, aux_z, out, out2, out3, n, D, H, W, Cout, ldo, epilogue, false, stream);
}

extern "C" int forge_wino_output_half(const float* Mm8, const float* Mm2_8, long long bs2, long long pt2, const float* bias, const float* scale, const float* shift, float slope,
                                      const float* residual, const float* aux_h, const float* aux_z, float* out, float* out2, float* out3, int n, int D, int H, int W,
                                      int Cout, int ldo, int epilogue, forge_stream_t stream) {
    return wino_output_impl(Mm8, Mm2_8, bs2, pt2, bias, scale, shift, slope, residual, aux_h, aux_z, out, out2, out3, n, D, H, W, Cout, ldo, epilogue, true, stream);
}
```

forge_amd/flopmeter.py:

```python
import torch

from . import _lib
from .convops import WINO_FORMS


def _v(a):
    return a.value if hasattr(a, "value") else a


def _igemm(a):
    C1, C2 = _v(a[1]), _v(a[5])
    n, D, H, W, Cout, ntaps = _v(a[19]), _v(a[20]), _v(a[21]), _v(a[22]), _v(a[27]), _v(a[30])
    return 2.0 * n * D * H * W * Cout * ntaps * (C1 + C2)


def _wino_counter(form):
    def count(a):
        loops = _v(a[17]) if form.kloops is None else form.kloops
        return float(2 * 16 * _v(a[12]) * _v(a[13]) * _v(a[14]) * _v(a[15]) * _v(a[16]) * loops * (_v(a[1]) + _v(a[6])))
    return count


def _wgrad(a):
    return 2.0 * _v(a[11]) * _v(a[12]) * _v(a[13]) * _v(a[14]) * _v(a[19]) * _v(a[21]) * (_v(a[3]) + _v(a[7]))


def _wino_wgrad(a):
    return 2.0 * 16 * _v(a[10]) * _v(a[11]) * _v(a[12]) * _v(a[13]) * _v(a[14]) * _v(a[15]) * (_v(a[2]) + _v(a[6]))


def _attention(a):
    return 4.0 * _v(a[5]) * _v(a[6]) * _v(a[7]) * _v(a[8])


def _attention_lse(a):
    return 4.0 * _v(a[6]) * _v(a[7]) * _v(a[8]) * _v(a[9])


def _attention_bwd(a):
    dv = _v(a[9])
    return (16.0 if dv else 14.0) * _v(a[11]) * _v(a[12]) * _v(a[13]) * _v(a[14])


def _attention_mh(a):
    return 4.0 * _v(a[5]) * _v(a[6]) * _v(a[7]) * _v(a[8]) * _v(a[9])


def _attention_mh_bwd(a):
    return (16.0 if _v(a[8]) else 14.0) * _v(a[10]) * _v(a[11]) * _v(a[12]) * _v(a[13]) * _v(a[14])


def _token_fwd(a):
    return 2.0 * _v(a[13]) * _v(a[14]) * _v(a[15])


def _token_bwd(a):
    dxn = _v(a[9]) or _v(a[12]) or _v(a[13])
    return 2.0 * _v(a[16]) * _v(a[17]) * _v(a[18]) * ((1 if dxn else 0) + (1 if _v(a[10]) else 0))


_ENTRIES = {"forge_conv_igemm": _igemm, **{f.gemm: _wino_counter(f) for f in WINO_FORMS.values()}, "forge_conv_wgrad": _wgrad, "forge_wino_wgrad": _wino_wgrad,
            "forge_attention_fwd": _attention, "forge_attention_fwd_lse": _attention_lse, "forge_attention_bwd": _attention_bwd,
            "forge_attention_mh_fwd": _attention_mh, "forge_attention_mh_bwd": _attention_mh_bwd,
            "forge_token_linear_fwd": _token_fwd, "forge_token_linear_bwd": _token_bwd}
_wino_gemm, _wino_gemm_dn, _wino_gemm_dn4 = (_ENTRIES[WINO_FORMS[k].gemm] for k in ("points", "dn", "dn4"))


class FlopMeter:
    def __init__(self):
        self.flops = {k: 0.0 for k in _ENTRIES}
        self.launches = {k: 0 for k in _ENTRIES}

    def __enter__(self):
        self._lib = _lib.lib()
        self._orig = {}
        for name, fn in _ENTRIES.items():
            orig = getattr(self._lib, name)
            self._orig[name] = orig

            def wrapped(*a, _orig=orig, _fn=fn, _name=name):
                self.flops[_name] += _fn(a)
                self.launches[_name] += 1
                return _orig(*a)
            setattr(self._lib, name, wrapped)
        return self

    def __exit__(self, *exc):
        for name, orig in self._orig.items():
            setattr(self._lib, name, orig)
        return False

    @property
    def gflop(self):
        return sum(self.flops.values()) / 1e9

    def summary(self):
        return {"executed_gflop": self.gflop, "launches": dict(self.launches), "gflop_by_entry": {k: v / 1e9 for k, v in self.flops.items()}}


def stage_replay_ms(model, sample, dev, iters=20):
    from . import geo_utils
    from .graph import GraphedCall
    """{stage: ms per replay} for FORGE's inference step on `sample` (b scenes, 5 input views, V cameras)."""
    e3 = model.encoder_3d
    b = sample["images"].shape[0]
    t = 5
    with torch.no_grad():
        img = sample["images"][:, :t].reshape(b * t, 3, 256, 256).contiguous()
        lifted = e3._trunk_hip(img)
        feats = e3._conv1_hip(lifted).reshape(b, t, 128, 32, 32, 32)
        poses = sample["cam_poses_cv2_canonicalized"][:, :t].contiguous()
        rotated = model.rotate(voxels=feats, camPoses_cv2=poses, grid_size=32, order="distance")
        fused = e3.fuse(rotated)
        fv, dv = e3.heads(fused)
        V = sample["K_cv2"].shape[1]
        cams = geo_utils.camera_dict(sample["cam_extrinsics_cv2_canonicalized"], sample["K_cv2"])
        v2v = model._view2vol(b, V, dev)
    stages = {
        "encoder_resnet": lambda: e3._trunk_hip(img),
        "encoder_conv1": lambda: e3._conv1_hip(lifted),
        "rotate": lambda: model.rotate(voxels=feats, camPoses_cv2=poses, grid_size=32, order="distance"),
        "fuse": lambda: e3.fuse(rotated),
        "heads": lambda: e3.heads(fused),
        "render(+conv_rgb)": lambda: model.render(cams, fv, dv, return_origin_proj=True, view2vol=v2v),
    }
    out = {}
    for name, fn in stages.items():
        def call(fn=fn):
            with torch.no_grad():
                return fn()
        g = GraphedCall(call, dev, warmup=2)
        g()
        torch.cuda.synchronize()
        a, bq = torch.cuda.Event(enable_timing=True), torch.cuda.Event(enable_timing=True)
        a.record()
        for _ in range(iters):
            g()
        bq.record()
        torch.cuda.synchronize()
        out[name] = a.elapsed_time(bq) / iters
        del g
    return out
```

forge_amd/fusion.py:

```python
import torch
import torch.nn as nn

from . import _lib, convops as co, determinism


def hip_inference(module, x):
    return x.is_cuda and x.dtype == torch.float32 and not module.training and not torch.is_grad_enabled()


def frozen_eval(module, x):
    return (x.is_cuda and x.dtype == torch.float32 and not module.training and torch.is_grad_enabled()
            and not any(p.requires_grad for p in module.parameters()))


def affine_act_bwd(dy, y, scale, slope, out=None):
    C = dy.shape[-1]
    M = dy.numel() // C
    if out is None:
        out = torch.empty(dy.shape, dtype=torch.float32, device=dy.device)
    _lib.check(_lib.lib().forge_affine_act_bwd(_lib.ptr(dy), dy.stride(-2), _lib.ptr(y), y.stride(-2), _lib.ptr(scale), float(slope), _lib.ptr(out),
                                               out.stride(-2), M, C, _lib.current_stream()), "forge_affine_act_bwd")
    return out


# ... 90 lines not shown
    @_lib.on_tensor_device
    def forward(ctx, x, gamma, beta, running_mean, running_var, eps, slope, residual):
        M, C = x.shape
        L, p = _lib.lib(), _lib.ptr
        y = torch.empty(M, C, dtype=torch.float32, device=x.device)
        mean, invstd = torch.empty(C, dtype=torch.float32, device=x.device), torch.empty(C, dtype=torch.float32, device=x.device)
        res = None if residual is None else (residual if _rows_ok(residual, C) else residual.contiguous())
        _lib.check(L.forge_bn_eval_fwd(p(x), x.stride(0), p(gamma), p(beta), p(running_mean), p(running_var), float(eps), float(slope), p(y), C, p(mean),
                                       p(invstd), M, C, p(res), 0 if res is None else res.stride(0), _lib.current_stream()), "forge_bn_eval_fwd")
        ctx.save_for_backward(x, gamma, beta, mean, invstd, y if res is not None else None)
        ctx.slope = float(slope)
        return y

    @staticmethod
    @_lib.on_tensor_device
    def backward(ctx, dy):
        x, gamma, beta, mean, invstd, y = ctx.saved_tensors
        M, C = x.shape
        L, p, st = _lib.lib(), _lib.ptr, _lib.current_stream
        dy = dy if _rows_ok(dy, C) else dy.contiguous()
        dx = torch.empty(M, C, dtype=torch.float32, device=x.device)
        dres = torch.empty(M, C, dtype=torch.float32, device=x.device) if (y is not None and ctx.needs_input_grad[7]) else None
        dg = torch.empty(C, dtype=torch.float32, device=x.device) if gamma is not None else None
        db = torch.empty(C, dtype=torch.float32, device=x.device) if beta is not None else None
        if dg is not None or db is not None:
            ws = torch.empty(L.forge_bn_ws_doubles(C), dtype=torch.float64, device=x.device)
            _lib.check(L.forge_bn_sync_bwd_reduce(p(dy), dy.stride(0), p(x), x.stride(0), p(gamma), p(beta), p(mean), p(invstd), ctx.slope, p(dg), p(db), p(ws),
                                                  M, C, p(y), C, st()), "forge_bn_sync_bwd_reduce")
        zero = torch.zeros(2 * C, dtype=torch.float64, device=x.device)
        _lib.check(L.forge_bn_sync_bwd_apply(p(dy), dy.stride(0), p(x), x.stride(0), p(gamma), p(beta), p(mean), p(invstd), ctx.slope, p(dx), C, p(zero),
                                             M, M, C, p(y), C, p(dres), C, st()), "forge_bn_sync_bwd_apply")
        return dx, dg, db, None, None, None, None, dres


def _sync_world(bn):
    import torch.distributed as tdist
    if not (isinstance(bn, nn.SyncBatchNorm) and tdist.is_available() and tdist.is_initialized()):
        return 1
    return tdist.get_world_size(bn.process_group)


def _bn_group(bn):
    if _sync_world(bn) <= 1:
        return None
    import torch.distributed as tdist
    return bn.process_group if bn.process_group is not None else tdist.group.WORLD


def bn_hip_train(bn, rows):
    return (bn.training and rows.is_cuda and rows.dtype == torch.float32 and rows.shape[-1] % 4 == 0
            and (bn.momentum is not None or not bn.track_running_stats))


def bn_module_args(bn):
    track = bn.track_running_stats and bn.running_mean is not None
    return (bn.running_mean if track else None, bn.running_var if track else None, bn.momentum if bn.momentum is not None else 0.0, bn.eps,
            bn.num_batches_tracked if (track and bn.num_batches_tracked is not None) else None, _bn_group(bn))


def bn_act_rows(bn, rows, slope=1.0, residual=None, stats=None):
    C = rows.shape[-1]
    require_hip_input("BatchNorm on channels-last rows", rows)
    if C % 4:
        raise RuntimeError("forge_amd: the HIP BatchNorm kernels need a channel count that is a multiple of 4 (got %d)" % C)
    if bn.training and bn.momentum is None and bn.track_running_stats:
        raise RuntimeError("forge_amd: BatchNorm with momentum=None (cumulative moving average) is not implemented by the HIP kernels "
                           "(the reference's modules use the default momentum 0.1)")
    if not bn.training and bn.track_running_stats and bn.running_mean is not None:
        x = rows.reshape(-1, C)
        x = x if _rows_ok(x, C) else x.contiguous()
        res = None if residual is None else residual.reshape(-1, C)
        return _BNEvalRows.apply(x, bn.weight, bn.bias, bn.running_mean, bn.running_var, bn.eps, slope, res).reshape(rows.shape)
    if bn_hip_train(bn, rows) or not bn.track_running_stats or bn.running_mean is None:
        x = rows.reshape(-1, C)
        x = x if _rows_ok(x, C) else x.contiguous()
        rm, rv, mom, eps, nbt, group = bn_module_args(bn)
        res = None if residual is None else residual.reshape(-1, C)
        args = (x, bn.weight, bn.bias, rm, rv, mom, eps, slope, res, nbt)
        y = _BNTrainRows.apply(*args, group, stats if (stats is not None and stats.numel() and x.data_ptr() == rows.data_ptr()) else None)
        return y.reshape(rows.shape)
    raise RuntimeError("forge_amd: unsupported BatchNorm configuration %r" % (bn,))


def _step_scratch(R, C, dev, form=None):
    F = co.WINO_FORMS
    P2, P1 = ((form or F["half" if co.wino_half_applies(R, c, C) else "points"]).P for c in (2 * C, C))
    return torch.empty(max(P2 * 2 * C, P1 * C) * R, dtype=torch.float32, device=dev)


def require_hip_input(what, x, channels=None):
    if not (torch.is_tensor(x) and x.is_cuda and x.dtype == torch.float32):
        raise RuntimeError("forge_amd: %s runs only on the MI355X HIP kernels and needs a float32 tensor on a cuda/HIP device (got %s on %s); "
                           "there is no CPU or stock-PyTorch path" % (what, getattr(x, "dtype", type(x)), getattr(x, "device", "?")))
    if channels is not None and channels % 32:
        raise RuntimeError("forge_amd: %s needs a channel count that is a multiple of the GEMM K-step 32 (got %d)" % (what, channels))


class _GRUCellRows(torch.autograd.Function):

    @staticmethod
    @_lib.on_tensor_device
    def forward(ctx, x, h, wg, bg, wo, bo):
        b, D, H, W, C = h.shape
        Cx = x.shape[-1]
        M = b * D * H * W
        dev = h.device
        h = h.contiguous()
        wgc, woc = wg.detach().contiguous(), wo.detach().contiguous()
        bsx = co._batch_stride_rows(x)
        grid = (b, D, H, W)
        new = lambda c: torch.empty(b, D, H, W, c, dtype=torch.float32, device=dev)
        g = new(2 * C)
        co.conv3_launch(x, Cx, h, C, wgc, bg, g, grid, 2 * C, bs1=bsx)
        z, r, hr = new(C), new(C), new(C)
        L, p, st = _lib.lib(), _lib.ptr, _lib.current_stream
        _lib.check(L.forge_gru_gates_fwd(p(g), p(h), p(z), p(r), p(hr), M, C, st()), "forge_gru_gates_fwd")
        cand = new(C)
        co.conv3_launch(x, Cx, hr, C, woc, bo, cand, grid, C, bs1=bsx)
        hn = new(C)
        _lib.check(L.forge_gru_state_fwd(p(cand), p(h), p(z), p(hn), M, C, st()), "forge_gru_state_fwd")
        ctx.save_for_backward(x, h, z, r, hr, cand, wgc, woc)
        ctx.has_bias = (bg is not None, bo is not None)
        return hn

    @staticmethod
    @_lib.on_tensor_device
    def backward(ctx, dhn):
        x, h, z, r, hr, cand, wg, wo = ctx.saved_tensors
        b, D, H, W, C = h.shape
        Cx = x.shape[-1]
        M = b * D * H * W
        dev = h.device
        grid = (b, D, H, W)
        bsx = co._batch_stride_rows(x)
        new = lambda c: torch.empty(b, D, H, W, c, dtype=torch.float32, device=dev)
        L, p, st = _lib.lib(), _lib.ptr, _lib.current_stream
        dhn = dhn.contiguous()
        dh, dz, dc = new(C), new(C), new(C)
        _lib.check(L.forge_gru_state_bwd(p(dhn), C, p(h), p(z), p(cand), p(dh), p(dz), p(dc), M, C, None, 0, 0, 0, st()), "forge_gru_state_bwd")
        dxh = new(Cx + C)
        co.conv3_launch(dc, C, None, 0, wo, None, dxh, grid, Cx + C, dgrad=True)
        dwo = dbo = dwg = dbg = None
        if ctx.needs_input_grad[4]:
            dwo = co.grad_zeros(wo.shape, wo.device)
            co.conv3_wgrad(dc, x, Cx, hr, C, dwo, grid, C, bs1=bsx)
        if ctx.has_bias[1] and ctx.needs_input_grad[5]:
            dbo = co.colsum(dc.reshape(M, C))
        dg = new(2 * C)
        _lib.check(L.forge_gru_gates_bwd(p(dz), _lib.ptr(dxh[..., Cx:]), Cx + C, p(h), p(z), p(r), p(dg), p(dh), None, 0, M, C, None, 0, 0, 0, st()), "forge_gru_gates_bwd")
        dxh2 = new(Cx + C)
        co.conv3_launch(dg, 2 * C, None, 0, wg, None, dxh2, grid, Cx + C, dgrad=True)
        if ctx.needs_input_grad[2]:
            dwg = co.grad_zeros(wg.shape, wg.device)
            co.conv3_wgrad(dg, x, Cx, h, C, dwg, grid, 2 * C, bs1=bsx)
        if ctx.has_bias[0] and ctx.needs_input_grad[3]:
            dbg = co.colsum(dg.reshape(M, 2 * C))
        dx = (dxh[..., :Cx] + dxh2[..., :Cx]) if ctx.needs_input_grad[0] else None
        dh_total = (dh + dxh2[..., Cx:]) if ctx.needs_input_grad[1] else None
        return dx, dh_total, dwg, dbg, dwo, dbo


class _GRUCellPreRows(torch.autograd.Function):

    @staticmethod
    @_lib.on_tensor_device
    def forward(ctx, gx, cx, h, wgh, bg, woh, bo):
        b, D, H, W, C = h.shape
        M = b * D * H * W
        dev = h.device
        h, gx, cx = h.contiguous(), gx.contiguous(), cx.contiguous()
# ... 13 lines not shown
        ctx.has_bias = (bg is not None, bo is not None)
        return hn

    @staticmethod
    @_lib.on_tensor_device
    def backward(ctx, dhn):
        h, z, r, hr, cand, wg, wo = ctx.saved_tensors
        b, D, H, W, C = h.shape
        M = b * D * H * W
        dev = h.device
        grid = (b, D, H, W)
        new = lambda c: torch.empty(b, D, H, W, c, dtype=torch.float32, device=dev)
        L, p, st = _lib.lib(), _lib.ptr, _lib.current_stream
        dhn = dhn.contiguous()
        dh, dz, dc = new(C), new(C), new(C)
        _lib.check(L.forge_gru_state_bwd(p(dhn), C, p(h), p(z), p(cand), p(dh), p(dz), p(dc), M, C, None, 0, 0, 0, st()), "forge_gru_state_bwd")
        dhr = new(C)
        co.conv3_launch(dc, C, None, 0, wo, None, dhr, grid, C, dgrad=True)
        dwo = dbo = dwg = dbg = None
        if ctx.needs_input_grad[5]:
            dwo = co.grad_zeros(wo.shape, wo.device)
            co.conv3_wgrad(dc, hr, C, None, 0, dwo, grid, C)
        if ctx.has_bias[1] and ctx.needs_input_grad[6]:
            dbo = co.colsum(dc.reshape(M, C))
        dg = new(2 * C)
        _lib.check(L.forge_gru_gates_bwd(p(dz), p(dhr), C, p(h), p(z), p(r), p(dg), p(dh), None, 0, M, C, None, 0, 0, 0, st()), "forge_gru_gates_bwd")
        dh_total = new(C)
        co.conv3_launch(dg, 2 * C, None, 0, wg, None, dh_total, grid, C, residual=dh, dgrad=True)
        if ctx.needs_input_grad[3]:
            dwg = co.grad_zeros(wg.shape, wg.device)
            co.conv3_wgrad(dg, h, C, None, 0, dwg, grid, 2 * C)
        if ctx.has_bias[0] and ctx.needs_input_grad[4]:
            dbg = co.colsum(dg.reshape(M, 2 * C))
        return (dg if ctx.needs_input_grad[0] else None), (dc if ctx.needs_input_grad[1] else None), dh_total, dwg, dbg, dwo, dbo


def view_run(g):
    g = list(g)
    return g == list(range(g[0], g[0] + len(g)))


def _view_mean(xr, grp):
    C = xr.shape[-1]
    if view_run(grp):
        return xr[:, grp[0]:grp[0] + len(grp)].mean(dim=1).reshape(-1, C)
    return torch.stack([xr[:, ti] for ti in grp], dim=1).mean(dim=1).reshape(-1, C)


def _wino_view_mean(xr, grp, out):
    b, t, D, H, W, C = xr.shape
    vol = D * H * W
    if view_run(grp):
        return co.wino_input(xr[:, grp[0]:], C, C, b, D, H, W, bs=t * vol, out=out, nsum=len(grp), sum_stride=vol)
    return co.wino_input(_view_mean(xr, grp), C, C, b, D, H, W, out=out)


def _input_products(Vx, U, n, geo, Cout):
    b, D, H, W = geo
    C = Vx.shape[-1]
    R = b * D * (H // 2) * (W // 2)
    return co.wino_gemm(Vx, C, None, 0, U, None, n, D, H // 2, W // 2, Cout, half=co.wino_half_applies(R, Cout, C))


def _h0_wino(p, xr, grp, V, Mm, t0, h, wk="_U"):
    b, t, D, H, W, C = xr.shape
    gemm = lambda k: co.wino_gemm(V, C, None, 0, p[k + wk], Mm, b, D, H // 2, W // 2, C)
    _wino_view_mean(xr, grp, V)
    Mp = gemm("fc0")
    co.wino_output(Mp, p["fc0_b"], *p["bn1"], 0.01, None, None, None, t0, None, None, b, D, H, W, C, C, co.EPI_AFFINE_ACT)
    co.wino_input(t0, C, C, b, D, H, W, out=V)
    Mp = gemm("fc3")
    co.wino_output(Mp, p["fc3_b"], *p["bn4"], 0.01, None, None, None, h, None, None, b, D, H, W, C, C, co.EPI_AFFINE_ACT)


def _h0_direct(p, xr, grp, t0, h):
    b, t, D, H, W, C = xr.shape
    grid, taps = (b, D, H, W), co.TAPS_3x3x3
    co.conv_igemm(_view_mean(xr, grp), C, C, None, 0, 0, p["fc0_w"], p["fc0_b"], *p["bn1"], 0.01, None, None, None, t0, None, grid, grid[1:], C, C,
                  taps, epilogue=co.EPI_AFFINE_ACT)
    co.conv_igemm(t0, C, C, None, 0, 0, p["fc3_w"], p["fc3_b"], *p["bn4"], 0.01, None, None, None, h, None, grid, grid[1:], C, C, taps,
                  epilogue=co.EPI_AFFINE_ACT)


def _wino_step(geo, x, view, views, wg, wo, V, Mm, h, z, hr, hn, out=None, r=None, cand=None, calls=None):
    b, D, H, W = geo
    C = h.shape[-1]
    transform, gemm = calls or co.wino_calls(co.WINO_FORMS["points"])

    def conv(src, U, Cout, i):
        Vs = transform(src, C, C, b, D, H, W, out=V)
        if isinstance(x, tuple):
            return Vs, gemm(Vs, C, None, 0, U, Mm, b, D, H // 2, W // 2, Cout), dict(Mm2=x[i], view=view, views=views)
        return Vs, gemm(x, C, Vs, C, U, Mm, b, D, H // 2, W // 2, Cout, view=view, views=views), {}

    Vh, G, add = conv(h, wg[0], 2 * C, 0)
    co.wino_output(G, wg[1], None, None, 1.0, None, h, None, z, hr, r, *geo, 2 * C, C, co.EPI_GRU_GATES, **add)
    Vhr, S, add = conv(hr, wo[0], C, 1)
    co.wino_output(S, *wo[1:], 1.0, None, h, z, hn, out, cand, *geo, C, C, co.EPI_GRU_OUT, **add)
    return Vh, Vhr


def _direct_step(grid, x, wg, wo, h, z, hr, hn, out=None, r=None, cand=None, bs=0):
    C = h.shape[-1]
    ig, taps = grid[1:], co.TAPS_3x3x3
    split = isinstance(x, tuple)
    operands = lambda src, i: ((src, C, C, None, 0, 0), x[i]) if split else ((x, C, C, src, C, C), None)
    ops, res = operands(h, 0)
    co.conv_igemm(*ops, *wg, None, None, 1.0, res, h, None, z, hr, grid, ig, 2 * C, C, taps, epilogue=co.EPI_GRU_GATES, bs1=bs, out3=r)
    ops, res = operands(hr, 1)
    co.conv_igemm(*ops, *wo, 1.0, res, h, z, hn, out, grid, ig, C, C, taps, epilogue=co.EPI_GRU_OUT, bs1=bs, out3=cand)


_WKEY = {None: "_U", co.WINO_FORMS["dn"]: "_Ud", co.WINO_FORMS["dn4"]: "_Ud4"}
_PACKS = ((None, ("gate", "out", "fc0", "fc3")), (co.WINO_FORMS["dn"], ("gate", "out", "fc0", "fc3")), (co.WINO_FORMS["dn4"], ("gate", "out")))


def _fuse_eval(gru, xr, groups, wino, split, h0=None, keep=None, const0=None):
    b, t, D, H, W, C = xr.shape
    dev, M, vol = xr.device, b * D * H * W, D * H * W
    geo = (b, D, H, W)
    new = lambda c=C: torch.empty(M, c, dtype=torch.float32, device=dev)
    step, conv0 = None, None
    if wino:
        R = b * D * (H // 2) * (W // 2)
        F = co.WINO_FORMS
        both = lambda form: all(form.applies(R, D, H // 2, W // 2, c, 2 * C) for c in (2 * C, C))
        if not split and keep is None and const0 is None and both(F["dn"]):
            step = F["dn4"] if both(F["dn4"]) and co.wino_fits(b, D, H, W, C, views=t, form=F["dn4"]) else F["dn"]
            conv0 = F["dn"] if F["dn"].applies(R, D, H // 2, W // 2, C, C) else None
    p = gru._packed_halves(wino) if (split or const0 is not None) else gru._packed_wino(step) if wino else gru._packed()
    wk = _WKEY[step] if wino else "_w"
    weights = lambda half: ((p["gate" + wk + half], p["gate_b"]), (p["out" + wk + half], p["out_b"], *p["norm"]))
    wg, wo = weights("h" if split else "")
    if wino:
        calls = co.wino_calls(step or F["points"])
        X = calls[0](xr, C, C, b * t, D, H, W)
        if split:
            X = (_input_products(X, p["gate_Ux"], b * t, geo, 2 * C), _input_products(X, p["out_Ux"], b * t, geo, C))
        Vs = torch.empty(16, int(R * (step.rows if step else 1)), C, dtype=torch.float32, device=dev)
        V = Vs.reshape(-1)[:16 * R * C].view(16, R, C)
        Mm = _step_scratch(R, C, dev, step)
    elif split:
        X = {}
        for ti in sorted({ti for g in groups for ti in g}):
            X[ti] = (new(2 * C), new())
            for k, dst in zip(("gate_wx", "out_wx"), X[ti]):
                co.conv_igemm(xr[:, ti], C, C, None, 0, 0, p[k], None, None, None, 1.0, None, None, None, dst, None, geo, geo[1:], dst.shape[1],
                              dst.shape[1], co.TAPS_3x3x3, epilogue=co.EPI_BIAS, bs1=t * vol)
    outs = []
    for grp in groups:
        grp = list(grp)
        t0, h, out = new(), new(), new()
        if h0 is not None:
            h.copy_(h0.permute(0, 2, 3, 4, 1).reshape(M, C))
        elif wino:
            _h0_wino(p, xr, grp, V, Mm, t0, h, _WKEY[conv0])
        else:
            _h0_direct(p, xr, grp, t0, h)
        if keep is not None:
            keep.append(t0)
        if const0 is not None and "MXg0" not in const0:
            Vx0 = co.wino_input(xr[:, 0], C, C, b, D, H, W, bs=t * vol)
            const0["MXg0"], const0["MXc0"] = _input_products(Vx0, p["gate_Ux"], b, geo, 2 * C), _input_products(Vx0, p["out_Ux"], b, geo, C)
        z, hr, hn, r, cand = new(), new(), t0, None, None
        for k, ti in enumerate(grp):
            if keep is not None:
                z, hr, r, hn, cand = new(), new(), new(), new(), new()
            last = out if k == len(grp) - 1 else None
            if not wino:
                _direct_step(geo, X[ti] if split else xr[:, ti], wg, wo, h, z, hr, hn, last, r, cand, bs=0 if split else t * vol)
            elif const0 is not None and k == 0:
                _wino_step(geo, (const0["MXg0"], const0["MXc0"]), 0, 1, *weights("h"), V, Mm, h, z, hr, hn, last, r, cand)
            else:
                _wino_step(geo, X, ti, t, wg, wo, Vs, Mm, h, z, hr, hn, last, r, cand, calls=calls)
            if keep is not None:
                keep += [h, z, r, cand]
            h, hn = hn, h
        outs.append(out.reshape(b, D, H, W, C).permute(0, 4, 1, 2, 3))
    return outs


def _eval_chunks(x, fuse):
    b, t, C, D, H, W = x.shape
    xr = x.permute(0, 1, 3, 4, 5, 2)
    xr = xr if xr.is_contiguous() else xr.contiguous()
    nb = co.wino_scene_chunk(b, D, H, W, C, views=t) if co.wino_enabled() else 0
    parts = [fuse(xr[i:i + (nb or b)], nb > 0, i, i + (nb or b)) for i in range(0, b, nb or b)]
    return parts[0] if len(parts) == 1 else [torch.cat(o, dim=0) for o in zip(*parts)]


class _FuseFrozen(torch.autograd.Function):

    @staticmethod
    @_lib.on_tensor_device
    def forward(ctx, x, gru, skip_dx0=False, const0=None):
        ctx.skip_dx0 = bool(skip_dx0)
        b, t, C, D, H, W = x.shape
        xr = x.permute(0, 1, 3, 4, 5, 2)
        xr = xr if xr.is_contiguous() else xr.contiguous()
        wino = co.wino_enabled() and co.wino_fits(b, D, H, W, C, views=t)
        saved = []
        out = _fuse_eval(gru, xr, [range(t)], wino, False, keep=saved, const0=const0 if (wino and skip_dx0) else None)[0]
        ctx.gru, ctx.shape = gru, (b, t, C, D, H, W)
        ctx.save_for_backward(*saved)
        return out

    @staticmethod
    @_lib.on_tensor_device
    def backward(ctx, dout):
        gru = ctx.gru
        b, t, C, D, H, W = ctx.shape
        saved = ctx.saved_tensors
        t0, steps = saved[0], [saved[1 + 4 * i:5 + 4 * i] for i in range(t)]
        p = gru._packed_T()
        dev, M = dout.device, b * D * H * W
        grid = (b, D, H, W)
        new = lambda c=C: torch.empty(M, c, dtype=torch.float32, device=dev)
        L, ptr, st = _lib.lib(), _lib.ptr, _lib.current_stream
        dgrad = lambda dy, Cdy, k, dst, Cdst, residual=None: co.conv3_launch(dy, Cdy, None, 0, p[k + "_w"], None, dst, grid, Cdst, residual=residual,
                                                                           dgrad=True, U=p[k + "_UT"], wT=p[k + "_wT"])
        dr = dout.permute(0, 2, 3, 4, 1)
        dr = (dr if dr.is_contiguous() else dr.contiguous()).reshape(M, C)
        dhn = dr * p["norm_scale"]
        ld_dhn = C
        dx = torch.empty(b, t, D, H, W, C, dtype=torch.float32, device=dev)
        for ti in reversed(range(t)):
            h, z, r, cand = steps[ti]
            dh, dz, dc, dg = new(), new(), new(), new(2 * C)
            _lib.check(L.forge_gru_state_bwd(ptr(dhn), ld_dhn, ptr(h), ptr(z), ptr(cand), ptr(dh), ptr(dz), ptr(dc), M, C, None, 0, 0, 0, st()), "forge_gru_state_bwd")
            if ti == 0 and ctx.skip_dx0:
                dhr = dgrad(dc, C, "out_h", new(), C)
                dhp = new()
                _lib.check(L.forge_gru_gates_bwd(ptr(dz), ptr(dhr), C, ptr(h), ptr(z), ptr(r), ptr(dg), ptr(dh), ptr(dhp), C, M, C, None, 0, 0, 0, st()),
                           "forge_gru_gates_bwd")
                toth = dgrad(dg, 2 * C, "gate_h", new(), C, residual=dhp)
                dx[:, 0].zero_()
                dhn, ld_dhn = toth, C
                continue
            dxh = new(2 * C)
            dgrad(dc, C, "out", dxh, 2 * C)
            _lib.check(L.forge_gru_gates_bwd(ptr(dz), ptr(dxh[:, C:]), 2 * C, ptr(h), ptr(z), ptr(r), ptr(dg), ptr(dh), ptr(dxh[:, C:]), 2 * C, M, C,
                                             None, 0, 0, 0, st()), "forge_gru_gates_bwd")
            tot = new(2 * C)
            dgrad(dg, 2 * C, "gate", tot, 2 * C, residual=dxh)
            dx[:, ti] = tot.view(b, D, H, W, 2 * C)[..., :C]
            dhn, ld_dhn = tot[:, C:], 2 * C
        h0 = steps[0][0]
        g = torch.empty(M, C, dtype=torch.float32, device=dev)
        affine_act_bwd(dhn, h0, p["bn4_scale"], 0.01, out=g)
        g2 = new()
        dgrad(g, C, "fc3", g2, C)
        affine_act_bwd(g2, t0, p["bn1_scale"], 0.01, out=g)
        dgrad(g, C, "fc0", g2, C)
        dx.add_(g2.reshape(b, 1, D, H, W, C), alpha=1.0 / t)
        return dx.permute(0, 1, 5, 2, 3, 4), None, None, None


# ... 184 lines not shown
    def __init__(self, config, input_size, hidden_size):
        super().__init__()
        self.input_size = input_size
        self.hidden_size = hidden_size
        self.conv_gate = nn.Conv3d(input_size + hidden_size, hidden_size * 2, 3, padding=1)
        self.out_gate = nn.Conv3d(input_size + hidden_size, hidden_size, 3, padding=1)

    def forward(self, x, prev_state=None):
        require_hip_input("ConvGRUCell_3D", x, self.input_size)
        require_hip_input("ConvGRUCell_3D", x, self.hidden_size)
        b, c, d, h, w = x.shape
        if prev_state is None:
            prev_state = torch.zeros([b, self.hidden_size, d, h, w], dtype=x.dtype, device=x.device)
        rows = lambda v: v.permute(0, 2, 3, 4, 1).contiguous()
        hn = gru_cell_rows(rows(x), rows(prev_state), self.conv_gate.weight, self.conv_gate.bias, self.out_gate.weight, self.out_gate.bias)
        return hn.permute(0, 4, 1, 2, 3)


class ConvGRU_3D(co.PackedModule):

    def __init__(self, config, n_layers=1, input_size=16, hidden_size=16):
        super().__init__()
        self._pack_cache = co.PackCache()
        self.input_size = input_size
        self.hidden_size = hidden_size
        self.n_layers = n_layers
        self.cells = nn.ModuleList([
            ConvGRUCell_3D(config, input_size if i == 0 else hidden_size, hidden_size) for i in range(n_layers)])
        self.fusion_norm = nn.BatchNorm3d(hidden_size)
        self.fusion_conv = nn.Sequential(
            nn.Conv3d(input_size, input_size, 3, padding=1),
            nn.BatchNorm3d(input_size),
            nn.LeakyReLU(inplace=True),
            nn.Conv3d(input_size, input_size, 3, padding=1),
            nn.BatchNorm3d(input_size),
            nn.LeakyReLU(inplace=True),
        )

    def _packed(self):
        cell = self.cells[0]
        fc = self.fusion_conv
        src = [cell.conv_gate.weight, cell.conv_gate.bias, cell.out_gate.weight, cell.out_gate.bias,
               fc[0].weight, fc[0].bias, fc[3].weight, fc[3].bias] + \
              [t for bn in (fc[1], fc[4], self.fusion_norm) for t in (bn.weight, bn.bias, bn.running_mean, bn.running_var)]

        def build():
            return {
                "gate_w": co.pack_conv3d_weight(cell.conv_gate.weight), "gate_b": cell.conv_gate.bias.detach().contiguous(),
                "out_w": co.pack_conv3d_weight(cell.out_gate.weight), "out_b": cell.out_gate.bias.detach().contiguous(),
                "fc0_w": co.pack_conv3d_weight(fc[0].weight), "fc0_b": fc[0].bias.detach().contiguous(),
                "fc3_w": co.pack_conv3d_weight(fc[3].weight), "fc3_b": fc[3].bias.detach().contiguous(),
                "bn1": co.bn_affine(fc[1]), "bn4": co.bn_affine(fc[4]), "norm": co.bn_affine(self.fusion_norm),
            }
        return self._pack_cache.get(src, build)

    def _packed_T(self):
        p = self._packed()
        if "gate_wT" not in p:
            tr = lambda w: w.transpose(1, 2).contiguous()
            p.update({"gate_wT": tr(p["gate_w"]), "out_wT": tr(p["out_w"]), "fc0_wT": tr(p["fc0_w"]), "fc3_wT": tr(p["fc3_w"]),
                      "norm_scale": p["norm"][0], "bn1_scale": p["bn1"][0], "bn4_scale": p["bn4"][0]})
            p.update({k + "_UT": co.wino_pack_packed(p[k + "_w"], transpose=True) for k in ("gate", "out", "fc0", "fc3")})
            C = self.hidden_size
            for k in ("gate", "out"):
                p[k + "_h_w"] = p[k + "_w"][:, :, C:].contiguous()
                p[k + "_h_wT"] = p[k + "_h_w"].transpose(1, 2).contiguous()
                p[k + "_h_UT"] = p[k + "_UT"][:, :, C:, :].contiguous()
        return p

    def fuse_frozen_hip(self, x, skip_dx0=False, const0=None):
        assert self.n_layers == 1 and self.input_size == self.hidden_size
        require_hip_input("ConvGRU_3D.fuse_frozen_hip", x, x.shape[2])
        return _FuseFrozen.apply(x, self, bool(skip_dx0), const0)

    def fuse_hip(self, x, h0=None):
        assert self.n_layers == 1 and self.input_size == self.hidden_size
        require_hip_input("ConvGRU_3D.fuse_hip", x, x.shape[2])
        t = x.shape[1]
        return _eval_chunks(x, lambda xr, wino, i, j: _fuse_eval(self, xr, [range(t)], wino, False, h0=None if h0 is None else h0[i:j]))[0]

    def _packed_wino(self, form=None):
        p = self._packed()
        for f, convs in _PACKS:
            if convs[0] + _WKEY[f] not in p:
                p.update({k + _WKEY[f]: co.wino_pack(f or co.WINO_FORMS["points"], p[k + "_w"]) for k in convs})
            if f is form:
                break
        return p

    def _packed_halves(self, wino):
        p = self._packed_wino() if wino else self._packed()
        wk = "_U" if wino else "_w"
        if "gate" + wk + "x" not in p:
            C = self.hidden_size
            for k in ("gate", "out"):
                w = p[k + wk]
                p[k + wk + "x"], p[k + wk + "h"] = w[..., :C].contiguous(), w[..., C:].contiguous()
        return p

    def fuse_groups_hip(self, x, groups):
        assert self.n_layers == 1 and self.input_size == self.hidden_size
        require_hip_input("ConvGRU_3D.fuse_groups_hip", x, x.shape[2])
        return _eval_chunks(x, lambda xr, wino, i, j: _fuse_eval(self, xr, groups, wino, True))

    def fuse_autograd_hip(self, x):
        assert self.n_layers == 1
        require_hip_input("ConvGRU_3D.fuse_autograd_hip", x, x.shape[2])
        b, t, C, D, H, W = x.shape
        xr = x.permute(0, 1, 3, 4, 5, 2)
        xr = xr if xr.is_contiguous() else xr.contiguous()
        cell, fc = self.cells[0], self.fusion_conv
        lrelu = 0.01
        h = bn_act_rows(fc[1], co.conv3x3x3_rows(xr.mean(dim=1), None, fc[0].weight, fc[0].bias), lrelu)
        h = bn_act_rows(fc[4], co.conv3x3x3_rows(h, None, fc[3].weight, fc[3].bias), lrelu)
        for xv in xr.unbind(1):
            h = gru_cell_rows(xv, h, cell.conv_gate.weight, cell.conv_gate.bias, cell.out_gate.weight, cell.out_gate.bias)
        return bn_act_rows(self.fusion_norm, h).permute(0, 4, 1, 2, 3)

    def fuse_groups_autograd_hip(self, x, groups):
        assert self.n_layers == 1 and self.input_size == self.hidden_size
        require_hip_input("ConvGRU_3D.fuse_groups_autograd_hip", x, x.shape[2])
        b, t, C, D, H, W = x.shape
        cell, fc = self.cells[0], self.fusion_conv
        bns = (fc[1], fc[4], self.fusion_norm)
        rows_probe = x.permute(0, 1, 3, 4, 5, 2)
        if (co.wino_enabled() and co.wino_fits(b, D, H, W, 2 * C, views=t) and co.wino_wgrad_applies(b, D, H, W, C, 0, C)
                and all(bn_hip_train(m, rows_probe) and m.weight is not None for m in bns)
                and all(isinstance(a, nn.LeakyReLU) and a.negative_slope == 0.01 for a in (fc[2], fc[5]))):
            outs = _FuseGroupsTrain.apply(x, cell.conv_gate.weight, cell.conv_gate.bias, cell.out_gate.weight, cell.out_gate.bias,
                                          fc[0].weight, fc[0].bias, fc[1].weight, fc[1].bias, fc[3].weight, fc[3].bias, fc[4].weight, fc[4].bias,
                                          self.fusion_norm.weight, self.fusion_norm.bias, self, tuple(tuple(g) for g in groups))
            return list(outs)
        xt = x.permute(1, 0, 3, 4, 5, 2).contiguous()
        Wg, Wo = cell.conv_gate.weight, cell.out_gate.weight
        flat = xt.reshape(t * b, D, H, W, C)
        gx_all = co.conv3x3x3_rows(flat, None, Wg[:, :C], None).reshape(t, b, D, H, W, 2 * C).unbind(0)
        cx_all = co.conv3x3x3_rows(flat, None, Wo[:, :C], None).reshape(t, b, D, H, W, C).unbind(0)
        xviews = xt.unbind(0)
        wgh, woh = co._pack3d(Wg[:, C:]).contiguous(), co._pack3d(Wo[:, C:]).contiguous()
        lrelu = 0.01
        outs = []
        for grp in groups:
            grp = list(grp)
            xm = sum(xviews[ti] for ti in grp) / float(len(grp))
            h = bn_act_rows(fc[1], co.conv3x3x3_rows(xm, None, fc[0].weight, fc[0].bias), lrelu)
            h = bn_act_rows(fc[4], co.conv3x3x3_rows(h, None, fc[3].weight, fc[3].bias), lrelu)
            for ti in grp:
                h = _GRUCellPreRows.apply(gx_all[ti], cx_all[ti], h, wgh, cell.conv_gate.bias, woh, cell.out_gate.bias)
            outs.append(bn_act_rows(self.fusion_norm, h).permute(0, 4, 1, 2, 3))
        return outs

    def forward(self, x, hidden=None):
        require_hip_input("ConvGRU_3D", x, x.shape[2])
        if not hidden:
            hidden = [None] * self.n_layers
        if self.n_layers == 1 and hip_inference(self, x) and self.input_size == self.hidden_size:
            h0 = hidden[0]
            if h0 is None:
                h0 = torch.zeros(x.shape[0], self.hidden_size, *x.shape[3:], dtype=x.dtype, device=x.device)
            return self.fuse_hip(x, h0=h0)
        cur = x
        h = None
        for layer_idx in range(self.n_layers):
            h = hidden[layer_idx]
            outs = []
            for t in range(x.shape[1]):
# ... 7 lines not shown
```

include/forge_hip.h:

```cpp
#ifndef FORGE_HIP_H
#define FORGE_HIP_H

#ifdef __cplusplus
extern "C" {
#endif

typedef void* forge_stream_t;

#define FORGE_EINVAL (-1)
#define FORGE_ESHAPE (-2)

int forge_version(void);
const char* forge_last_error(void);

int forge_rotate_fwd(const float* vox, const float* xf, const int* mode, float* out,
                     int n, int C, int D, int H, int W, forge_stream_t stream);

int forge_rotate_fwd_slots(const float* vox, const float* xf, const int* mode, const int* dst_slot, float* out,
                           int n, int C, int D, int H, int W, forge_stream_t stream);

int forge_rotate_xf_from_poses(const float* poses, float* xf, int* mode, int* slot, const float* dist, int B, int t, float half_extent,
                               forge_stream_t stream);

int forge_pose_chain_fwd(const float* rot, const float* trans, const float* can_pose, const float* can_extr, const float* K, float half_extent,
                         int b, int t, float* xf, int* mode, int* slot, float* cam16, float* poses, float* origin, float* jac, forge_stream_t stream);
int forge_pose_chain_bwd(const float* jac, const float* dxf, const float* dcam, float* drot, float* dtrans, int b, int t, forge_stream_t stream);

int forge_rotate_bwd(const float* dout, const float* vox, const float* xf, const int* mode,
                     float* dvox, float* dxf, int n, int C, int D, int H, int W,
                     forge_stream_t stream);
int forge_rotate_bwd_slots(const float* dout, const float* vox, const float* xf, const int* mode, const int* src_slot,
                           float* dvox, float* dxf, int n, int C, int D, int H, int W, forge_stream_t stream);

int forge_render_fwd(const float* feat, const float* dens, const float* cam, const int* view2vol,
                     float* out_feat, float* out_opac, float* out_depth,
                     int V, int nvol, int C, int D, int H, int W, int Hr, int Wr, int S,
                     float zmin, float zmax, float hx, float hy, float hz,
                     forge_stream_t stream);

int forge_pack_cameras(const float* R, long long r0, long long r1, long long r2, const float* T, long long t0, long long t1,
                       const float* K, long long k0, long long k1, long long k2, float* cam16, float* origin, int V, forge_stream_t stream);

long long forge_render_bwd_ws_bytes(int V, int C, int Hr, int Wr, int S, int want_cam);
int forge_render_bwd(const float* feat, const float* dens, const float* cam, const int* view2vol,
                     const float* g_feat, const float* g_opac, const float* g_depth,
                     float* dfeat, float* ddens, float* dcam,
                     int V, int nvol, int C, int D, int H, int W, int Hr, int Wr, int S,
                     float zmin, float zmax, float hx, float hy, float hz,
                     void* ws, long long ws_bytes, forge_stream_t stream);

int forge_resize_bilinear_fwd(const float* in, float* out, int P, int Hi, int Wi, int Ho, int Wo, forge_stream_t stream);
int forge_resize_bilinear_bwd(const float* g, float* din, int P, int Hi, int Wi, int Ho, int Wo, forge_stream_t stream);

int forge_conv_igemm(const float* in1, int C1, int ld1, long long bs1, const float* in2, int C2, int ld2, long long bs2,
                     const float* wp,
                     const float* bias, const float* scale, const float* shift, float slope, const float* residual,
                     const float* aux_h, const float* aux_z, float* out, float* out2, float* out3,
                     int n, int D, int H, int W, int is, int Di, int Hi, int Wi, int Cout, int ldo,
                     const int* taps, int ntaps, int os, int pz, int py, int px, int Do, int Ho, int Wo,
                     int epilogue, int lift, int tile, int ksplit, float* splitk_ws, long long splitk_ws_bytes, double* stats, forge_stream_t stream);

int forge_conv_igemm_plan(long long M, int Cout, int Cin, int ntaps, int nphase, int epilogue, int ldo, long long splitk_ws_bytes,
                          int* tile, int* ksplit);

int forge_wino_weights(const float* wp, float* U, int Cout, int Cin, int kd, int transpose, forge_stream_t stream);
int forge_wino_dy(const float* dy, int ldy, float* dM, int n, int D, int H, int W, int Cout, forge_stream_t stream);
int forge_wino_wgrad(const float* dMm, const float* V1, int C1, long long bs1, long long pt1, const float* V2, int C2, long long bs2,
                     long long pt2, float* dU, int n, int D, int Ht, int Wt, int Cout, int kd, forge_stream_t stream);
int forge_wino_dw(const float* dU, float* dw, int Cout, int Cin, int kd, forge_stream_t stream);
int forge_wino_input(const float* in, int ld, long long bs, float* V, int ldv, long long ptv, int n, int D, int H, int W, int C,
                     int nsum , long long sum_stride,
                     forge_stream_t stream);
int forge_wino_input_dy(const float* dy, int ld, float* V, float* dM, int n, int D, int H, int W, int C, forge_stream_t stream);
int forge_wino_gemm(const float* V1, int C1, int ld1, long long bs1, long long pt1, const float* V2, int C2, int ld2, long long bs2,
                    long long pt2, const float* U, float* Mm, int n, int D, int Ht, int Wt, int Cout, int kd, int tile ,
                    forge_stream_t stream);
int forge_wino_gemm_half(const float* V1, int C1, int ld1, long long bs1, long long pt1, const float* V2, int C2, int ld2, long long bs2,
                         long long pt2, const float* U, float* Mm8, int n, int D, int Ht, int Wt, int Cout, int kd, forge_stream_t stream);
int forge_wino_output_half(const float* Mm8, const float* Mm2_8 , long long bs2, long long pt2, const float* bias, const float* scale,
                           const float* shift, float slope, const float* residual, const float* aux_h, const float* aux_z, float* out, float* out2, float* out3,
                           int n, int D, int H, int W, int Cout, int ldo, int epilogue, forge_stream_t stream);
int forge_wino_gemm_dn(const float* V1, int C1, int ld1, long long bs1, long long pt1, const float* V2, int C2, int ld2, long long bs2,
                       long long pt2, const float* Ud, float* Mm, int n, int D, int Ht, int Wt, int Cout, int kd, forge_stream_t stream);
int forge_wino_weights_dn(const float* wp, float* Ud, int Cout, int Cin, forge_stream_t stream);
int forge_wino_input_dn4(const float* in, int ld, long long bs, float* V6, int ldv, long long ptv, int n, int D, int H, int W, int C,
                         int nsum, long long sum_stride, forge_stream_t stream);
int forge_wino_weights_dn4(const float* wp, float* Ud, int Cout, int Cin, forge_stream_t stream);
int forge_wino_gemm_dn4(const float* V1, int C1, int ld1, long long bs1, long long pt1, const float* V2, int C2, int ld2, long long bs2,
                        long long pt2, const float* Ud, float* Mm, int n, int D, int Ht, int Wt, int Cout, int kd, forge_stream_t stream);
int forge_wino_gemm_tile(long long R, int Cout, int Cin);
int forge_wino_output(const float* Mm, const float* Mm2, long long bs2, long long pt2, const float* bias, const float* scale, const float* shift, float slope, const float* residual,
                      const float* aux_h, const float* aux_z, float* out, float* out2, float* out3, int n, int D, int H, int W, int Cout,
                      int ldo, int epilogue, forge_stream_t stream);

int forge_conv_wgrad(const float* dy, int ldy, const float* x1, int C1, int ld1, long long bs1, const float* x2, int C2, int ld2,
                     long long bs2, float* dw, int n, int D, int H, int W, int is, int Di, int Hi, int Wi, int Cout,
                     const int* taps, int ntaps, forge_stream_t stream);

int forge_conv_direct_fwd(const float* in, int ld_in, const float* w, const float* bias, float slope, float* out, int ld_out,
                          int n, int D, int H, int W, int Cin, int Cout, const int* taps, int ntaps, forge_stream_t stream);
int forge_conv_direct_dgrad(const float* dy, int ld_dy, const float* w, float* dx, int ld_dx,
                            int n, int D, int H, int W, int Cin, int Cout, const int* taps, int ntaps, forge_stream_t stream);
int forge_conv_direct_wgrad(const float* dy, int ld_dy, const float* x, int ld_x, float* dw,
                            int n, int D, int H, int W, int Cin, int Cout, const int* taps, int ntaps, forge_stream_t stream);

int forge_conv_wgrad_det(const float* dy, int ldy, const float* x1, int C1, int ld1, long long bs1, const float* x2, int C2, int ld2,
                         long long bs2, float* dw, int n, int D, int H, int W, int is, int Di, int Hi, int Wi, int Cout,
                         const int* taps, int ntaps, int accumulate, void* ws, long long ws_bytes, forge_stream_t stream);
long long forge_conv_wgrad_det_ws_bytes(int C1, int C2, int n, int D, int H, int W, int is, int Di, int Hi, int Wi, int Cout,
                                        const int* taps, int ntaps);
int forge_conv_wgrad_plan(int C1, int C2, int n, int D, int H, int W, int is, int Di, int Hi, int Wi, int Cout, const int* taps, int ntaps,
                          int det, long long* plan);
int forge_wino_wgrad_det(const float* dMm, const float* V1, int C1, long long bs1, long long pt1, const float* V2, int C2, long long bs2,
                         long long pt2, float* dU, int n, int D, int Ht, int Wt, int Cout, int kd, int accumulate, void* ws, long long ws_bytes,
                         forge_stream_t stream);
long long forge_wino_wgrad_det_ws_bytes(int C1, int C2, int n, int D, int Ht, int Wt, int Cout, int kd);
int forge_conv_direct_wgrad_det(const float* dy, int ld_dy, const float* x, int ld_x, float* dw, int n, int D, int H, int W, int Cin, int Cout,
                                const int* taps, int ntaps, int accumulate, void* ws, long long ws_bytes, forge_stream_t stream);
long long forge_conv_direct_wgrad_det_ws_bytes(int n, int D, int H, int W, int Cin, int Cout, int ntaps);
int forge_rotate_bwd_det(const float* dout, const float* vox, const float* xf, const int* mode, float* dvox, float* dxf,
                         int n, int C, int D, int H, int W, int accumulate, void* ws, long long ws_bytes, forge_stream_t stream);
long long forge_rotate_bwd_det_ws_bytes(int n, int C, int D, int H, int W);
int forge_rotate_bwd_slots_det(const float* dout, const float* vox, const float* xf, const int* mode, const int* src_slot,
                               float* dvox, float* dxf, int n, int C, int D, int H, int W, int accumulate, void* ws, long long ws_bytes,
                               forge_stream_t stream);
long long forge_rotate_bwd_slots_det_ws_bytes(int n, int C, int D, int H, int W);

int forge_gru_gates_fwd(const float* g, const float* h, float* z, float* r, float* hr, long long M, int C, forge_stream_t stream);
int forge_gru_state_fwd(float* c_cand, const float* h, const float* z, float* hn, long long M, int C, forge_stream_t stream);
int forge_gru_state_bwd(const float* dhn, int ld_dhn, const float* h, const float* z, const float* cand, float* dh, float* dz, float* dc,
                        long long M, int C, float* dc_acc, long long acc_bs, long long vol, int acc_mode, forge_stream_t stream);
int forge_gru_gates_bwd(const float* dz, const float* dhr, int ld_dhr, const float* h, const float* z, const float* r,
                        float* dg, float* dh, float* dh_out, int ld_dh_out, long long M, int C, float* dg_acc, long long acc_bs, long long vol,
                        int acc_mode, forge_stream_t stream);

int forge_bn_ws_doubles(int C);
int forge_colsum(const float* x, int ldx, float* out, double* ws, long long M, int C, forge_stream_t stream);
int forge_bn_train_fwd(const float* x, int ldx, const float* gamma, const float* beta, float eps, float slope, float* y, int ldy,
                       float* mean, float* invstd, float* running_mean, float* running_var, float momentum, double* ws,
                       long long M, int C, const float* res, int ldres, long long* num_batches_tracked,
                       int nblk_pre ,
                       forge_stream_t stream);
int forge_bn_train_bwd(const float* dy, int lddy, const float* x, int ldx, const float* gamma, const float* beta, const float* mean,
                       const float* invstd, float slope, float* dx, int lddx, float* dgamma, float* dbeta, double* ws, long long M, int C,
                       const float* y, int ldy, float* dres, int lddres, forge_stream_t stream);
int forge_bn_sync_stats(const float* x, int ldx, double* ws, long long M, int C, int nblk_pre , forge_stream_t stream);
int forge_bn_sync_fwd_apply(const float* x, int ldx, const float* gamma, const float* beta, float eps, float slope, float* y, int ldy,
                            float* mean, float* invstd, float* running_mean, float* running_var, float momentum, const double* totals,
                            long long M_total, long long M, int C, const float* res, int ldres, long long* num_batches_tracked, forge_stream_t stream);
int forge_bn_eval_fwd(const float* x, int ldx, const float* gamma, const float* beta, const float* running_mean, const float* running_var,
                      float eps, float slope, float* y, int ldy, float* mean, float* invstd, long long M, int C, const float* res, int ldres,
                      forge_stream_t stream);
int forge_bn_sync_bwd_reduce(const float* dy, int lddy, const float* x, int ldx, const float* gamma, const float* beta, const float* mean,
                             const float* invstd, float slope, float* dgamma, float* dbeta, double* ws, long long M, int C,
                             const float* y, int ldy, forge_stream_t stream);
int forge_bn_sync_bwd_apply(const float* dy, int lddy, const float* x, int ldx, const float* gamma, const float* beta, const float* mean,
                            const float* invstd, float slope, float* dx, int lddx, const double* totals, long long M_total, long long M, int C,
                            const float* y, int ldy, float* dres, int lddres, forge_stream_t stream);

int forge_affine_act_bwd(const float* dy, int ld_dy, const float* y, int ld_y, const float* scale, float slope, float* dx, int ld_dx,
                         long long M, int C, forge_stream_t stream);

int forge_attention_fwd(const float* q, const float* k, const float* v, long long v_batch_rows, float* out, int B, int Nq, int Nk, int d,
                        forge_stream_t stream);

int forge_attention_fwd_lse(const float* q, const float* k, const float* v, long long v_batch_rows, float* out, float* lse, int B, int Nq, int Nk,
                            int d, forge_stream_t stream);
int forge_attention_bwd(const float* q, const float* k, const float* v, long long v_batch_rows, const float* out, const float* lse,
                        const float* dout, float* dq, float* dk, float* dv, float* delta_ws, int B, int Nq, int Nk, int d, forge_stream_t stream);

int forge_attention_mh_fwd(const float* q, const float* k, const float* v, float* out, float* lse, int B, int H, int Nq, int Nk, int d,
                           long long q_bs, long long q_rs, long long k_bs, long long k_rs, long long v_bs, long long v_rs, long long out_bs,
// ... 76 lines not shown
```

Measured before the change: 928.6 views/s.

## Add F(4x2,3x3)x depth-nest Winograd form for ConvGRU 3D convolutions

Adds a new Winograd form, dn4h, for the ConvGRU gate and output convolutions. It uses an F(4,3) transform along height, giving 4-row tiles, in place of the F(2,3) 2-row tiles, on top of the existing depth-nest-4 scheme. The form has 24 transform points and its own input, weight, GEMM and output kernels. It is chosen by default when the shapes allow it. The aim is to cut the multiplies per output in the GRU convolutions. In exchange the transforms do more work and F(4,3) is less accurate numerically in fp32.

```diff
diff --git a/forge_amd/_lib.py b/forge_amd/_lib.py
--- a/forge_amd/_lib.py
+++ b/forge_amd/_lib.py
@@ -45,6 +45,10 @@
     "forge_wino_input_dn4": [_P, _I, _LL, _P, _I, _LL, _I, _I, _I, _I, _I, _I, _LL, _P],
     "forge_wino_weights_dn4": [_P, _P, _I, _I, _P],
     "forge_wino_gemm_dn4": [_P, _I, _I, _LL, _LL, _P, _I, _I, _LL, _LL, _P, _P, _I, _I, _I, _I, _I, _I, _P],
+    "forge_wino_input_dn4h": [_P, _I, _LL, _P, _I, _LL, _I, _I, _I, _I, _I, _I, _LL, _P],
+    "forge_wino_weights_dn4h": [_P, _P, _I, _I, _P],
+    "forge_wino_gemm_dn4h": [_P, _I, _I, _LL, _LL, _P, _I, _I, _LL, _LL, _P, _P, _I, _I, _I, _I, _I, _I, _P],
+    "forge_wino_output_dn4h": [_P, _P, _P, _P, _P, _P, _P, _P, _P, _I, _I, _I, _I, _I, _I, _I, _P],
     "forge_wino_output_half": [_P, _P, _LL, _LL, _P, _P, _P, _F, _P, _P, _P, _P, _P, _P, _I, _I, _I, _I, _I, _I, _I, _P],
     "forge_wino_gemm_tile": [_LL, _I, _I],
     "forge_wino_output": [_P, _P, _LL, _LL, _P, _P, _P, _F, _P, _P, _P, _P, _P, _P, _I, _I, _I, _I, _I, _I, _I, _P],
diff --git a/forge_amd/convops.py b/forge_amd/convops.py
--- a/forge_amd/convops.py
+++ b/forge_amd/convops.py
@@ -199,6 +199,7 @@
     winograd = True
     wino_depth_nest = os.environ.get("FORGE_WINO_DEPTH_NEST", "1") != "0"
     wino_depth_nest4 = os.environ.get("FORGE_WINO_DEPTH_NEST4", "1") != "0"
+    wino_h4 = os.environ.get("FORGE_WINO_H4", "1") != "0"
 
 
 STATE = _State()
@@ -421,8 +422,9 @@
 
 
 def wino_fits(n, D, H, W, C, views=1, nest4=False, form=None):
-    rows = n * views * D * (H // 2) * (W // 2) * (form or WINO_FORMS["dn4" if nest4 else "points"]).rows
-    return H % 2 == 0 and W % 2 == 0 and rows * C * 4 <= MAX_OPERAND_BYTES
+    form = form or WINO_FORMS["dn4" if nest4 else "points"]
+    rows = n * views * D * (H // form.th) * (W // 2) * form.rows
+    return H % form.th == 0 and W % 2 == 0 and rows * C * 4 <= MAX_OPERAND_BYTES
 
 
 @_lib.on_tensor_device
@@ -447,7 +449,11 @@
     return STATE.wino_depth_nest4 and D % 4 == 0 and D >= 8 and wino_depth_nest_applies(R, D, Ht, Wt, Cout, Cin)
 
 
-WinoForm = collections.namedtuple("WinoForm", "name P gemm weights ushape input rows kloops applies tile metered")
+def wino_depth_nest4h_applies(R, D, Ht, Wt, Cout, Cin):
+    return STATE.wino_h4 and wino_depth_nest4_applies(R, D, Ht, Wt, Cout, Cin)
+
+
+WinoForm = collections.namedtuple("WinoForm", "name P gemm weights ushape input rows kloops applies tile metered points th", defaults=(16, 2))
 _U4 = lambda kd, co_, ci_: (16, kd, co_, ci_)
 WINO_FORMS = {f.name: f for f in (
     WinoForm("points", 16, "forge_wino_gemm", "forge_wino_weights", _U4, "forge_wino_input", 1, None, lambda R, D, Ht, Wt, Cout, Cin: True,
@@ -459,6 +465,9 @@
     WinoForm("dn4", 16, "forge_wino_gemm_dn4", "forge_wino_weights_dn4", lambda kd, co_, ci_: (16, 6, co_, ci_), "forge_wino_input_dn4", Fraction(3, 2),
              Fraction(3, 2), lambda *a: wino_depth_nest4_applies(*a), False, False),
 )}
+
+WINO_DN4H = WinoForm("dn4h", 24, "forge_wino_gemm_dn4h", "forge_wino_weights_dn4h", lambda kd, co_, ci_: (24, 6, co_, ci_), "forge_wino_input_dn4h",
+                     Fraction(3, 2), Fraction(3, 2), lambda *a: wino_depth_nest4h_applies(*a), False, False, 24, 4)
 
 
 def wino_calls(form):
@@ -484,10 +493,10 @@
 
 @_lib.on_tensor_device
 def wino_form_input(form, x, C, ld, n, D, H, W, bs=0, out=None, nsum=1, sum_stride=0):
-    rows = int(n * D * (H // 2) * (W // 2) * form.rows)
-    V = out if out is not None else torch.empty(16, rows, C, dtype=torch.float32, device=x.device)
-    if form.rows != 1 and (V.shape != (16, rows, C) or not V.is_contiguous()):
-        raise ValueError("depth-nest operand buffer %s is not [16][%d][%d]" % (tuple(V.shape), rows, C))
+    rows = int(n * D * (H // form.th) * (W // 2) * form.rows)
+    V = out if out is not None else torch.empty(form.points, rows, C, dtype=torch.float32, device=x.device)
+    if form.rows != 1 and (V.shape != (form.points, rows, C) or not V.is_contiguous()):
+        raise ValueError("depth-nest operand buffer %s is not [%d][%d][%d]" % (tuple(V.shape), form.points, rows, C))
     _lib.check(getattr(_lib.lib(), form.input)(_lib.ptr(x), ld, int(bs), _lib.ptr(V), C, 0, n, D, H, W, C, int(nsum), int(sum_stride), _lib.current_stream()),
                form.input)
     return V
@@ -547,10 +556,17 @@
 
 @_lib.on_tensor_device
 def wino_output(Mm, bias, scale, shift, slope, residual, aux_h, aux_z, out, out2, out3, n, D, H, W, Cout, ldo, epilogue, Mm2=None, view=0, views=1):
-    vol = D * (H // 2) * (W // 2)
     P = Mm.shape[0] if Mm.dim() == 3 else 0
-    if P not in (8, 16) or Mm.shape[1:] != (n * vol, Cout) or not Mm.is_contiguous():
-        raise ValueError("point products %s do not match [8 | 16][%d][%d]" % (tuple(Mm.shape), n * vol, Cout))
+    vol = D * (H // (WINO_DN4H.th if P == WINO_DN4H.P else 2)) * (W // 2)
+    if P not in (8, 16, WINO_DN4H.P) or Mm.shape[1:] != (n * vol, Cout) or not Mm.is_contiguous():
+        raise ValueError("point products %s do not match [8 | 16][%d][%d] (or the 24 points' rows)" % (tuple(Mm.shape), n * vol, Cout))
+    if P == WINO_DN4H.P:
+        if Mm2 is not None or residual is not None or H % 4 or epilogue not in (EPI_GRU_GATES, EPI_GRU_OUT):
+            raise ValueError("24-point products take the GRU tails only, without a second addend or a residual, on H %% 4 == 0 (H=%d epilogue=%d)" % (H, epilogue))
+        _lib.check(_lib.lib().forge_wino_output_dn4h(_lib.ptr(Mm), _lib.ptr(bias), _lib.ptr(scale), _lib.ptr(shift), _lib.ptr(aux_h), _lib.ptr(aux_z),
+                                                     _lib.ptr(out), _lib.ptr(out2), _lib.ptr(out3), n, D, H, W, Cout, ldo, epilogue, _lib.current_stream()),
+                   "forge_wino_output_dn4h")
+        return out
     if Mm2 is not None and (Mm2.shape != (P, n * views * vol, Cout) or not Mm2.is_contiguous()):
         raise ValueError("second addend %s does not match [%d][%d][%d] (the form of Mm)" % (tuple(Mm2.shape), P, n * views * vol, Cout))
     p2 = None if Mm2 is None else ctypes.c_void_p(Mm2.data_ptr() + 4 * view * vol * Cout)
diff --git a/forge_amd/csrc/conv_igemm.hip b/forge_amd/csrc/conv_igemm.hip
--- a/forge_amd/csrc/conv_igemm.hip
+++ b/forge_amd/csrc/conv_igemm.hip
@@ -1139,7 +1139,8 @@
 
 static int wino_gemm_impl(const float* V1, int C1, int ld1, long long bs1, long long pt1, const float* V2, int C2, int ld2, long long bs2,
                           long long pt2, const float* U, float* Mm, int n, int D, int Ht, int Wt, int Cout, int kd, int tile, int form, forge_stream_t stream) {
-    const bool half = form == 1, dn = form == 2, dn4 = form == 3;
+    const bool half = form == 1, dn = form == 2, dn4h = form == 4, dn4 = form == 3 || dn4h;
+    const char* const name4 = dn4h ? "forge_wino_gemm_dn4h" : "forge_wino_gemm_dn4";
     FORGE_REQUIRE(tile == 0 || (tile >= 'A' && tile <= 'E'), FORGE_EINVAL, "forge_wino_gemm: tile must be 0 (default rule) or 'A'..'E'");
     FORGE_REQUIRE(V1 && U && Mm && (kd == 1 || kd == 3), FORGE_EINVAL, "forge_wino_gemm: null pointer argument / kd not 1 or 3");
     FORGE_REQUIRE(n > 0 && D > 0 && Ht > 0 && Wt > 0 && Cout > 16, FORGE_EINVAL, "forge_wino_gemm: bad dims n=%d D=%d Ht=%d Wt=%d Cout=%d (Cout > 16)", n,
@@ -1150,7 +1151,8 @@
     FORGE_REQUIRE(!dn || (kd == 3 && D % 2 == 0 && ((long long)Ht * Wt) % 64 == 0), FORGE_EINVAL,
                   "forge_wino_gemm_dn: needs three depth taps, an even D and Ht Wt %% 64 == 0 (kd=%d D=%d Ht=%d Wt=%d)", kd, D, Ht, Wt);
     FORGE_REQUIRE(!dn4 || (kd == 3 && D % 4 == 0 && ((long long)Ht * Wt) % 64 == 0), FORGE_EINVAL,
-                  "forge_wino_gemm_dn4: needs three depth taps, D %% 4 == 0 and Ht Wt %% 64 == 0 (kd=%d D=%d Ht=%d Wt=%d)", kd, D, Ht, Wt);
+                  "%s: needs three depth taps, D %% 4 == 0 and Ht Wt %% 64 == 0 (kd=%d D=%d Ht=%d Wt=%d)", name4, kd, D, Ht, Wt);
+    FORGE_REQUIRE(!dn4h || D >= 8, FORGE_EINVAL, "forge_wino_gemm_dn4h: D=%d must be at least 8", D);
     ConvArgs a;
     memset(&a, 0, sizeof(a));
     const long long vol = (long long)D * Ht * Wt, R = (long long)n * vol, rows = dn4 ? vol / 4 * 6 : vol, Cin = C1 + C2;
@@ -1160,7 +1162,7 @@
     a.span2 = V2 ? ((long long)(n - 1) * a.bs2r + rows) * ld2 * 4 : 0;
     if (dn4) {
         FORGE_REQUIRE(a.span1 < (1ll << 31) && a.span2 < (1ll << 31) && R * Cout * 4 < (1ll << 31) && 6ll * Cout * Cin * 4 < (1ll << 31), FORGE_EINVAL,
-                      "forge_wino_gemm_dn4: an operand or an output plane spans >= 2 GiB (32-bit buffer offsets); split the batch");
+                      "%s: an operand or an output plane spans >= 2 GiB (32-bit buffer offsets); split the batch", name4);
     } else {
         FORGE_REQUIRE(a.span1 < (1ll << 31) && a.span2 < (1ll << 31) && R < (1ll << 31), FORGE_ESHAPE,
                       "forge_wino_gemm: an operand spans >= 2 GiB per Winograd point (32-bit buffer offsets); split the batch");
@@ -1169,15 +1171,15 @@
     }
     a.wp = U; a.slope = 1.f; a.out = Mm; a.n = n; a.D = D; a.H = Ht; a.W = Wt; a.is = 1; a.Di = D; a.Hi = Ht; a.Wi = Wt;
     a.Cout = Cout; a.ldo = Cout; a.ldr = Cout; a.ntaps = a.tpp = npos; a.os = 1; a.Do = D; a.Ho = Ht; a.Wo = Wt; a.nphase = 1; a.epi = EPI_BIAS;
-    a.ksplit = 1; a.nbat = half ? 4 : 16;
+    a.ksplit = 1; a.nbat = half ? 4 : dn4h ? 24 : 16;
     a.pt1 = pt1 > 0 ? pt1 : (long long)n * rows * ld1; a.pt2 = V2 ? (pt2 > 0 ? pt2 : (long long)n * rows * ld2) : 0;
     a.ptw = (long long)npos * Cout * Cin; a.pto = R * Cout;
     if (form == 0 || half) {
         if (kd == 3) { a.tap[0][0] = -1; a.tap[2][0] = 1; }
         if (!tile) tile = forge_wino_gemm_tile(R, Cout, C1 + C2);
     }
-    if (int rc = launch_conv_tile(a, (char)tile, (hipStream_t)stream, form)) return rc;
-    FORGE_LAUNCH_CHECK(dn4 ? "forge_wino_gemm_dn4" : dn ? "forge_wino_gemm_dn" : "forge_wino_gemm");
+    if (int rc = launch_conv_tile(a, (char)tile, (hipStream_t)stream, dn4h ? 3 : form)) return rc;
+    FORGE_LAUNCH_CHECK(dn4 ? name4 : dn ? "forge_wino_gemm_dn" : "forge_wino_gemm");
     return 0;
 }
 
@@ -1202,3 +1204,9 @@
     FORGE_REQUIRE(C1 > 0 && C1 % BK == 0 && C2 >= 0 && C2 % BK == 0, FORGE_EINVAL, "forge_wino_gemm_dn4: C1=%d / C2=%d must be multiples of %d", C1, C2, BK);
     return wino_gemm_impl(V1, C1, ld1, bs1, pt1, V2, C2, ld2, bs2, pt2, Ud, Mm, n, D, Ht, Wt, Cout, kd, 'B', 3, stream);
 }
+
+extern "C" int forge_wino_gemm_dn4h(const float* V1, int C1, int ld1, long long bs1, long long pt1, const float* V2, int C2, int ld2, long long bs2,
+                                    long long pt2, const float* Ud, float* Mm, int n, int D, int Ht, int Wt, int Cout, int kd, forge_stream_t stream) {
+    FORGE_REQUIRE(C1 > 0 && C1 % BK == 0 && C2 >= 0 && C2 % BK == 0, FORGE_EINVAL, "forge_wino_gemm_dn4h: C1=%d / C2=%d must be multiples of %d", C1, C2, BK);
+    return wino_gemm_impl(V1, C1, ld1, bs1, pt1, V2, C2, ld2, bs2, pt2, Ud, Mm, n, D, Ht, Wt, Cout, kd, 'B', 4, stream);
+}
diff --git a/forge_amd/csrc/winograd.hip b/forge_amd/csrc/winograd.hip
--- a/forge_amd/csrc/winograd.hip
+++ b/forge_amd/csrc/winograd.hip
@@ -6,6 +6,19 @@
 __device__ __forceinline__ float4 sub(float4 a, float4 b) { return make_float4(a.x - b.x, a.y - b.y, a.z - b.z, a.w - b.w); }
 __device__ __forceinline__ float add(float a, float b) { return a + b; }
 __device__ __forceinline__ float sub(float a, float b) { return a - b; }
+__device__ __forceinline__ float4 fma4(float k, float4 a, float4 b) { return make_float4(fmaf(k, a.x, b.x), fmaf(k, a.y, b.y), fmaf(k, a.z, b.z), fmaf(k, a.w, b.w)); }
+
+__device__ __forceinline__ void f43_six_lines(float p0, float p1, float p2, float p3, float p4, float p5, float& q0, float& q1, float& q2, float& q3, float& q4,
+                                              float& q5) {
+    const float a02 = p0 - p2, a24 = p2 - p4, s34 = p3 + p4, s12 = p1 + p2, d43 = p4 - p3, d12 = p1 - p2;
+    const float d42 = p4 - p2, d31 = p3 - p1, d13 = p1 - p3, d35 = p3 - p5;
+    q0 = fmaf(4.f, a02, -a24);
+    q1 = fmaf(-4.f, s12, s34);
+    q2 = fmaf(4.f, d12, d43);
+    q3 = fmaf(2.f, d31, d42);
+    q4 = fmaf(-2.f, d31, d42);
+    q5 = fmaf(4.f, d13, -d35);
+}
 
 __device__ __forceinline__ void tile_decode(long long idx, int per, int cs, int Ht, int Wt, unsigned& r, int& c, int& tw, int& th, unsigned& t) {
     r = (unsigned)(idx / per);
@@ -16,6 +29,14 @@
     th = (int)(q - t * (unsigned)Ht);
 }
 
+template <typename T>
+__device__ __forceinline__ void bt_cols_store(const T (&w)[4], float* vp, int i, long long ptv) {
+    *reinterpret_cast<T*>(vp + (4 * i + 0) * ptv) = sub(w[0], w[2]);
+    *reinterpret_cast<T*>(vp + (4 * i + 1) * ptv) = add(w[1], w[2]);
+    *reinterpret_cast<T*>(vp + (4 * i + 2) * ptv) = sub(w[2], w[1]);
+    *reinterpret_cast<T*>(vp + (4 * i + 3) * ptv) = sub(w[1], w[3]);
+}
+
 template <typename T, typename I>
 __device__ __forceinline__ void bt_d_b_store(const T (&d)[4][4], float* V, I row, int ld, int c, long long ptv) {
     T w[4][4];
@@ -28,12 +49,7 @@
     }
     float* vp = V + (long long)row * ld + c;
 #pragma unroll
-    for (int i = 0; i < 4; ++i) {
-        *reinterpret_cast<T*>(vp + (4 * i + 0) * ptv) = sub(w[i][0], w[i][2]);
-        *reinterpret_cast<T*>(vp + (4 * i + 1) * ptv) = add(w[i][1], w[i][2]);
-        *reinterpret_cast<T*>(vp + (4 * i + 2) * ptv) = sub(w[i][2], w[i][1]);
-        *reinterpret_cast<T*>(vp + (4 * i + 3) * ptv) = sub(w[i][1], w[i][3]);
-    }
+    for (int i = 0; i < 4; ++i) bt_cols_store(w[i], vp, i, ptv);
 }
 
 __device__ __forceinline__ void a_y_at_store(float4 y00, float4 y01, float4 y10, float4 y11, float* mp, long long ptm) {
@@ -48,17 +64,23 @@
     }
 }
 
+__device__ __forceinline__ double depth_row_f23(int k, double w0, double w1, double w2) {
+    return k == 0 ? w0 : k == 1 ? 0.5 * (w0 + w1 + w2) : k == 2 ? 0.5 * (w0 - w1 + w2) : w2;
+}
+__device__ __forceinline__ double depth_row_f43(int k, double w0, double w1, double w2) {
+    return k == 0 ? 0.25 * w0 : k == 1 ? -((w0 + w2) + w1) / 6.0 : k == 2 ? -((w0 + w2) - w1) / 6.0
+         : k == 3 ? ((0.25 * w0 + w2) + 0.5 * w1) / 6.0 : k == 4 ? ((0.25 * w0 + w2) - 0.5 * w1) / 6.0 : w2;
+}
+
+template <int NH = 4, double (*HROW)(int, double, double, double) = depth_row_f23>
 __device__ __forceinline__ void g_d_gt_store(const double (&d)[3][3], float* up, long long pt) {
-    double g[4][3];
-#pragma unroll
-    for (int b = 0; b < 3; ++b) {
-        g[0][b] = d[0][b];
-        g[1][b] = 0.5 * (d[0][b] + d[1][b] + d[2][b]);
-        g[2][b] = 0.5 * (d[0][b] - d[1][b] + d[2][b]);
-        g[3][b] = d[2][b];
-    }
-#pragma unroll
-    for (int i = 0; i < 4; ++i) {
+    double g[NH][3];
+#pragma unroll
+    for (int b = 0; b < 3; ++b)
+#pragma unroll
+        for (int i = 0; i < NH; ++i) g[i][b] = HROW(i, d[0][b], d[1][b], d[2][b]);
+#pragma unroll
+    for (int i = 0; i < NH; ++i) {
         up[(4 * i + 0) * pt] = (float)g[i][0];
         up[(4 * i + 1) * pt] = (float)(0.5 * (g[i][0] + g[i][1] + g[i][2]));
         up[(4 * i + 2) * pt] = (float)(0.5 * (g[i][0] - g[i][1] + g[i][2]));
@@ -111,8 +133,10 @@
     bt_d_b_store(d, a.V, r, a.ldv, c, a.ptv);
 }
 
+template <int TH>
 __global__ __launch_bounds__(256) void wino_input_dn4_kernel(const WinoInArgs a) {
-    const int Ht = a.H >> 1, Wt = a.W >> 1, Dg = a.D >> 2;
+    constexpr int NR = TH + 2;
+    const int Ht = TH == 4 ? a.H >> 2 : a.H >> 1, Wt = a.W >> 1, Dg = a.D >> 2;
     const long long idx = (long long)xcd_remap(blockIdx.x, gridDim.x) * 256 + threadIdx.x;
     const long long RG = (long long)a.n * Dg * Ht * Wt;
     if (idx >= RG * a.C) return;
@@ -124,10 +148,10 @@
     const long long HW = (long long)a.H * a.W;
     const float* base = a.in + (long long)t * a.bs * a.ld + c;
     const float inv = 1.f / (float)a.nsum;
-    float d[6][4][4];
-#pragma unroll
-    for (int i = 0; i < 4; ++i) {
-        const int y = 2 * th - 1 + i;
+    float d[6][NR][4];
+#pragma unroll
+    for (int i = 0; i < NR; ++i) {
+        const int y = TH * th - 1 + i;
 #pragma unroll
         for (int j = 0; j < 4; ++j) {
             const int x = 2 * tw - 1 + j;
@@ -147,20 +171,24 @@
                 }
                 p[e] = v;
             }
-            const float a02 = p[0] - p[2], a24 = p[2] - p[4], s34 = p[3] + p[4], s12 = p[1] + p[2], d43 = p[4] - p[3], d12 = p[1] - p[2];
-            const float d42 = p[4] - p[2], d31 = p[3] - p[1], d13 = p[1] - p[3], d35 = p[3] - p[5];
-            d[0][i][j] = fmaf(4.f, a02, -a24);
-            d[1][i][j] = fmaf(-4.f, s12, s34);
-            d[2][i][j] = fmaf(4.f, d12, d43);
-            d[3][i][j] = fmaf(2.f, d31, d42);
-            d[4][i][j] = fmaf(-2.f, d31, d42);
-            d[5][i][j] = fmaf(4.f, d13, -d35);
+            f43_six_lines(p[0], p[1], p[2], p[3], p[4], p[5], d[0][i][j], d[1][i][j], d[2][i][j], d[3][i][j], d[4][i][j], d[5][i][j]);
         }
     }
     const long long HWt = (long long)Ht * Wt;
     float* vp = a.V + ((((long long)t * Dg + g) * 6) * HWt + (long long)th * Wt + tw) * a.ldv + c;
-#pragma unroll
-    for (int k = 0; k < 6; ++k) bt_d_b_store(d[k], vp, k * HWt, a.ldv, 0, a.ptv);
+    if constexpr (TH == 4) {
+#pragma unroll
+        for (int k = 0; k < 6; ++k) {
+#pragma unroll
+            for (int j = 0; j < 4; ++j)
+                f43_six_lines(d[k][0][j], d[k][1][j], d[k][2][j], d[k][3][j], d[k][4][j], d[k][5][j], d[k][0][j], d[k][1][j], d[k][2][j], d[k][3][j], d[k][4][j], d[k][5][j]);
+#pragma unroll
+            for (int i = 0; i < 6; ++i) bt_cols_store(d[k][i], vp + k * HWt * a.ldv, i, a.ptv);
+        }
+    } else {
+#pragma unroll
+        for (int k = 0; k < 6; ++k) bt_d_b_store(d[k], vp, k * HWt, a.ldv, 0, a.ptv);
+    }
 }
 
 __global__ __launch_bounds__(256) void wino_weight_kernel(const float* __restrict__ wp, float* __restrict__ U, int Cout, int Cin, int KD, int transpose) {
@@ -181,15 +209,7 @@
     g_d_gt_store(w, U + ((long long)kd * No + o) * Nc + c, KD * per);
 }
 
-__device__ __forceinline__ double depth_row_f23(int k, double w0, double w1, double w2) {
-    return k == 0 ? w0 : k == 1 ? 0.5 * (w0 + w1 + w2) : k == 2 ? 0.5 * (w0 - w1 + w2) : w2;
-}
-__device__ __forceinline__ double depth_row_f43(int k, double w0, double w1, double w2) {
-    return k == 0 ? 0.25 * w0 : k == 1 ? -((w0 + w2) + w1) / 6.0 : k == 2 ? -((w0 + w2) - w1) / 6.0
-         : k == 3 ? ((0.25 * w0 + w2) + 0.5 * w1) / 6.0 : k == 4 ? ((0.25 * w0 + w2) - 0.5 * w1) / 6.0 : w2;
-}
-
-template <int K, double (*ROW)(int, double, double, double)>
+template <int K, double (*ROW)(int, double, double, double), int NH = 4, double (*HROW)(int, double, double, double) = depth_row_f23>
 __global__ __launch_bounds__(256) void wino_weight_nest_kernel(const float* __restrict__ wp, float* __restrict__ U, int Cout, int Cin) {
     const long long idx = (long long)blockIdx.x * 256 + threadIdx.x, per = (long long)Cout * Cin;
     if (idx >= per) return;
@@ -203,7 +223,7 @@
         for (int a = 0; a < 3; ++a)
 #pragma unroll
             for (int b = 0; b < 3; ++b) d[a][b] = ROW(k, w[0][a][b], w[1][a][b], w[2][a][b]);
-        g_d_gt_store(d, U + k * per + idx, K * per);
+        g_d_gt_store<NH, HROW>(d, U + k * per + idx, K * per);
     }
 }
 
@@ -236,17 +256,31 @@
     }
 }
 
-template <int EPI, bool HALF = false>
+template <int EPI, bool HALF = false, int TH = 2>
 __global__ __launch_bounds__(256) void wino_output_kernel(const WinoOutArgs a) {
-    const int C4 = a.Cout >> 2, Ht = a.H >> 1, Wt = a.W >> 1;
+    static_assert(TH == 2 || (TH == 4 && !HALF), "tiles of 2 x 2 voxels, or of 4 x 2 from the 24 points");
+    const int C4 = a.Cout >> 2, Ht = TH == 4 ? a.H >> 2 : a.H >> 1, Wt = a.W >> 1;
     const long long idx = (long long)blockIdx.x * 256 + threadIdx.x;
     const long long R = (long long)a.n * a.D * Ht * Wt;
     if (idx >= R * C4) return;
     unsigned r, t;
     int c, tw, th;
     tile_decode(idx, C4, 2, Ht, Wt, r, c, tw, th, t);
-    float4 s[2][4];
-    if constexpr (HALF) {
+    float4 s[TH][4];
+    if constexpr (TH == 4) {
+        const float* mp = a.Mm + (long long)r * a.Cout + c;
+#pragma unroll
+        for (int j = 0; j < 4; ++j) {
+            float4 m[6];
+#pragma unroll
+            for (int i = 0; i < 6; ++i) m[i] = *reinterpret_cast<const float4*>(mp + (4 * i + j) * a.ptm);
+            const float4 sl = add(m[1], m[2]), dl = sub(m[1], m[2]), Sl = add(m[3], m[4]), Dl = sub(m[3], m[4]);
+            s[0][j] = add(add(sl, Sl), m[0]);
+            s[1][j] = fma4(2.f, Dl, dl);
+            s[2][j] = fma4(4.f, Sl, sl);
+            s[3][j] = add(fma4(8.f, Dl, dl), m[5]);
+        }
+    } else if constexpr (HALF) {
         load_planes<2>(s, a.Mm, a.ptm, a.Mm2, a.ptm2, a.bs2, a.Cout, (unsigned)(a.D * Ht * Wt), r, c);
     } else {
         float4 m[4][4];
@@ -257,9 +291,9 @@
             s[1][j] = sub(sub(m[1][j], m[2][j]), m[3][j]);
         }
     }
-    float4 y[2][2];
-#pragma unroll
-    for (int i = 0; i < 2; ++i) {
+    float4 y[TH][2];
+#pragma unroll
+    for (int i = 0; i < TH; ++i) {
         y[i][0] = add(add(s[i][0], s[i][1]), s[i][2]);
         y[i][1] = sub(sub(s[i][1], s[i][2]), s[i][3]);
     }
@@ -272,10 +306,10 @@
     const int Ch = a.Cout >> 1;
     const long long plane = (long long)t * a.H * a.W;
 #pragma unroll
-    for (int i = 0; i < 2; ++i)
+    for (int i = 0; i < TH; ++i)
 #pragma unroll
         for (int j = 0; j < 2; ++j) {
-            const long long orow = plane + (long long)(2 * th + i) * a.W + (2 * tw + j);
+            const long long orow = plane + (long long)(TH * th + i) * a.W + (2 * tw + j);
             float v[4] = {y[i][j].x + bias.x, y[i][j].y + bias.y, y[i][j].z + bias.z, y[i][j].w + bias.w};
             if (a.residual) {
                 const float4 rr = *reinterpret_cast<const float4*>(a.residual + orow * a.Cout + c);
@@ -420,14 +454,21 @@
     return wino_weights_launch("forge_wino_weights_dn4", wino_weight_nest_kernel<6, depth_row_f43>, (long long)Cout * Cin, stream, wp, Ud, Cout, Cin);
 }
 
-enum WinoInKind { IN_PLAIN, IN_DN4, IN_DY };
+extern "C" int forge_wino_weights_dn4h(const float* wp, float* Ud, int Cout, int Cin, forge_stream_t stream) {
+    FORGE_REQUIRE(wp && Ud && Cout > 0 && Cin > 0, FORGE_EINVAL, "forge_wino_weights_dn4h: bad argument");
+    return wino_weights_launch("forge_wino_weights_dn4h", wino_weight_nest_kernel<6, depth_row_f43, 6, depth_row_f43>, (long long)Cout * Cin, stream, wp, Ud, Cout, Cin);
+}
+
+enum WinoInKind { IN_PLAIN, IN_DN4, IN_DY, IN_DN4H };
 
 static int wino_input_impl(const char* name, WinoInKind kind, const float* in, int ld, long long bs, float* V, int ldv, long long ptv, float* dM, int n, int D, int H,
                            int W, int C, int nsum, long long sum_stride, forge_stream_t stream) {
-    const bool dn4 = kind == IN_DN4;
+    const bool dn4 = kind == IN_DN4 || kind == IN_DN4H;
+    const int th = kind == IN_DN4H ? 4 : 2;
     FORGE_REQUIRE(in && V && (kind != IN_DY || dM), FORGE_EINVAL, "%s: null pointer argument", name);
     FORGE_REQUIRE(nsum >= 1 && (nsum == 1 || sum_stride > 0), FORGE_EINVAL, "%s: nsum >= 1, and a positive sum_stride (rows) with nsum > 1", name);
     FORGE_REQUIRE(!dn4 || (D > 0 && D % 4 == 0), FORGE_EINVAL, "%s: D=%d must be a multiple of 4", name, D);
+    FORGE_REQUIRE(kind != IN_DN4H || (D >= 8 && H > 0 && H % 4 == 0), FORGE_EINVAL, "%s: D=%d H=%d (D >= 8; H a multiple of 4)", name, D, H);
     const bool ok = n > 0 && D > 0 && H > 0 && W > 0 && H % 2 == 0 && W % 2 == 0 && C > 0 && C % 4 == 0 && ld >= C && ld % 4 == 0 && ldv >= C && ldv % 4 == 0;
     if (kind == IN_DY)
         FORGE_REQUIRE(ok, FORGE_ESHAPE, "%s: n=%d D=%d H=%d W=%d C=%d ld=%d (H, W even; C, ld multiples of 4)", name, n, D, H, W, C, ld);
@@ -435,14 +476,15 @@
     WinoInArgs a;
     a.in = in; a.ld = ld; a.bs = bs > 0 ? bs : (long long)D * H * W; a.V = V; a.ldv = ldv; a.n = n; a.D = D; a.H = H; a.W = W; a.C = C;
     a.nsum = nsum; a.ss = sum_stride;
-    const long long R = (long long)n * (dn4 ? D / 4 : D) * (H / 2) * (W / 2), rows = dn4 ? 6 * R : R;
+    const long long R = (long long)n * (dn4 ? D / 4 : D) * (H / th) * (W / 2), rows = dn4 ? 6 * R : R;
     a.ptv = ptv > 0 ? ptv : rows * ldv;
     a.dM = dM; a.ptm = dM ? R * C : 0;
     FORGE_REQUIRE(rows < (1ll << 31), FORGE_ESHAPE, dn4 ? "%s: more than 2^31 operand rows; split the batch" : "%s: more than 2^31 tiles; split the batch", name);
     const long long total = R * (dn4 ? C : C / 4), grid = (total + 255) / 256;
     FORGE_REQUIRE(grid < (1ll << 31), FORGE_ESHAPE, "%s: grid too large", name);
     const dim3 g((unsigned)grid), b(256);
-    if (dn4) hipLaunchKernelGGL(wino_input_dn4_kernel, g, b, 0, (hipStream_t)stream, a);
+    if (kind == IN_DN4H) hipLaunchKernelGGL(wino_input_dn4_kernel<4>, g, b, 0, (hipStream_t)stream, a);
+    else if (dn4) hipLaunchKernelGGL(wino_input_dn4_kernel<2>, g, b, 0, (hipStream_t)stream, a);
     else if (kind == IN_DY) hipLaunchKernelGGL(wino_input_kernel<true>, g, b, 0, (hipStream_t)stream, a);
     else hipLaunchKernelGGL(wino_input_kernel<false>, g, b, 0, (hipStream_t)stream, a);
     FORGE_LAUNCH_CHECK(name);
@@ -457,6 +499,11 @@
 extern "C" int forge_wino_input_dn4(const float* in, int ld, long long bs, float* V6, int ldv, long long ptv, int n, int D, int H, int W, int C,
                                     int nsum, long long sum_stride, forge_stream_t stream) {
     return wino_input_impl("forge_wino_input_dn4", IN_DN4, in, ld, bs, V6, ldv, ptv, nullptr, n, D, H, W, C, nsum, sum_stride, stream);
+}
+
+extern "C" int forge_wino_input_dn4h(const float* in, int ld, long long bs, float* V, int ldv, long long ptv, int n, int D, int H, int W, int C,
+                                     int nsum, long long sum_stride, forge_stream_t stream) {
+    return wino_input_impl("forge_wino_input_dn4h", IN_DN4H, in, ld, bs, V, ldv, ptv, nullptr, n, D, H, W, C, nsum, sum_stride, stream);
 }
 
 extern "C" int forge_wino_input_dy(const float* dy, int ld, float* V, float* dM, int n, int D, int H, int W, int C, forge_stream_t stream) {
@@ -516,3 +563,28 @@
                                       int Cout, int ldo, int epilogue, forge_stream_t stream) {
     return wino_output_impl(Mm8, Mm2_8, bs2, pt2, bias, scale, shift, slope, residual, aux_h, aux_z, out, out2, out3, n, D, H, W, Cout, ldo, epilogue, true, stream);
 }
+
+extern "C" int forge_wino_output_dn4h(const float* Mm, const float* bias, const float* scale, const float* shift, const float* aux_h, const float* aux_z, float* out,
+                                      float* out2, float* out3, int n, int D, int H, int W, int Cout, int ldo, int epilogue, forge_stream_t stream) {
+    FORGE_REQUIRE(Mm && out && aux_h, FORGE_EINVAL, "forge_wino_output_dn4h: null pointer argument");
+    FORGE_REQUIRE(n > 0 && D > 0 && H > 0 && W > 0 && H % 4 == 0 && W % 2 == 0 && Cout > 0 && Cout % 8 == 0 && ldo % 4 == 0, FORGE_ESHAPE,
+                  "forge_wino_output_dn4h: n=%d D=%d H=%d W=%d Cout=%d ldo=%d (H multiple of 4, W even; Cout multiple of 8; ldo of 4)", n, D, H, W, Cout, ldo);
+    FORGE_REQUIRE(epilogue == W_GRU_GATES || epilogue == W_GRU_OUT, FORGE_EINVAL, "forge_wino_output_dn4h: epilogue %d is not a GRU tail (2, 3)", epilogue);
+    FORGE_REQUIRE(epilogue == W_GRU_GATES ? ldo == Cout / 2 : ldo >= Cout, FORGE_ESHAPE,
+                  "forge_wino_output_dn4h: ldo=%d (epilogue 3: ldo >= Cout=%d; epilogue 2: ldo == Cout / 2)", ldo, Cout);
+    FORGE_REQUIRE(epilogue != W_GRU_GATES || out2, FORGE_EINVAL, "forge_wino_output_dn4h: GRU gate epilogue needs out2");
+    FORGE_REQUIRE(epilogue != W_GRU_OUT || (aux_z && (!out2 || (scale && shift))), FORGE_EINVAL,
+                  "forge_wino_output_dn4h: GRU out epilogue needs aux_z (and scale/shift with out2)");
+    WinoOutArgs a;
+    const long long R = (long long)n * D * (H / 4) * (W / 2);
+    a.Mm = Mm; a.ptm = R * Cout; a.Mm2 = nullptr; a.bs2 = 0; a.ptm2 = 0; a.bias = bias; a.scale = scale; a.shift = shift; a.slope = 1.f; a.residual = nullptr;
+    a.aux_h = aux_h; a.aux_z = aux_z; a.out = out; a.out2 = out2; a.out3 = out3; a.ldo = ldo; a.n = n; a.D = D; a.H = H; a.W = W; a.Cout = Cout; a.epi = epilogue;
+    FORGE_REQUIRE(R < (1ll << 31), FORGE_ESHAPE, "forge_wino_output_dn4h: more than 2^31 tiles; split the batch");
+    const long long total = R * (Cout / 4), grid = (total + 255) / 256;
+    FORGE_REQUIRE(grid < (1ll << 31), FORGE_ESHAPE, "forge_wino_output_dn4h: grid too large");
+    const dim3 g((unsigned)grid), b(256);
+    if (epilogue == W_GRU_GATES) hipLaunchKernelGGL((wino_output_kernel<W_GRU_GATES, false, 4>), g, b, 0, (hipStream_t)stream, a);
+    else hipLaunchKernelGGL((wino_output_kernel<W_GRU_OUT, false, 4>), g, b, 0, (hipStream_t)stream, a);
+    FORGE_LAUNCH_CHECK("forge_wino_output_dn4h");
+    return 0;
+}
diff --git a/forge_amd/flopmeter.py b/forge_amd/flopmeter.py
--- a/forge_amd/flopmeter.py
+++ b/forge_amd/flopmeter.py
@@ -1,7 +1,7 @@
 import torch
 
 from . import _lib
-from .convops import WINO_FORMS
+from .convops import WINO_DN4H, WINO_FORMS
 
 
 def _v(a):
@@ -17,7 +17,7 @@
 def _wino_counter(form):
     def count(a):
         loops = _v(a[17]) if form.kloops is None else form.kloops
-        return float(2 * 16 * _v(a[12]) * _v(a[13]) * _v(a[14]) * _v(a[15]) * _v(a[16]) * loops * (_v(a[1]) + _v(a[6])))
+        return float(2 * form.points * _v(a[12]) * _v(a[13]) * _v(a[14]) * _v(a[15]) * _v(a[16]) * loops * (_v(a[1]) + _v(a[6])))
     return count
 
 
@@ -59,7 +59,7 @@
     return 2.0 * _v(a[16]) * _v(a[17]) * _v(a[18]) * ((1 if dxn else 0) + (1 if _v(a[10]) else 0))
 
 
-_ENTRIES = {"forge_conv_igemm": _igemm, **{f.gemm: _wino_counter(f) for f in WINO_FORMS.values()}, "forge_conv_wgrad": _wgrad, "forge_wino_wgrad": _wino_wgrad,
+_ENTRIES = {"forge_conv_igemm": _igemm, **{f.gemm: _wino_counter(f) for f in (*WINO_FORMS.values(), WINO_DN4H)}, "forge_conv_wgrad": _wgrad, "forge_wino_wgrad": _wino_wgrad,
             "forge_attention_fwd": _attention, "forge_attention_fwd_lse": _attention_lse, "forge_attention_bwd": _attention_bwd,
             "forge_attention_mh_fwd": _attention_mh, "forge_attention_mh_bwd": _attention_mh_bwd,
             "forge_token_linear_fwd": _token_fwd, "forge_token_linear_bwd": _token_bwd}
diff --git a/forge_amd/fusion.py b/forge_amd/fusion.py
--- a/forge_amd/fusion.py
+++ b/forge_amd/fusion.py
@@ -196,10 +196,13 @@
     raise RuntimeError("forge_amd: unsupported BatchNorm configuration %r" % (bn,))
 
 
-def _step_scratch(R, C, dev, form=None):
+def _step_scratch(R, C, dev, form=None, conv0=None):
     F = co.WINO_FORMS
-    P2, P1 = ((form or F["half" if co.wino_half_applies(R, c, C) else "points"]).P for c in (2 * C, C))
-    return torch.empty(max(P2 * 2 * C, P1 * C) * R, dtype=torch.float32, device=dev)
+    P2, P1 = ((form or F["half" if co.wino_half_applies(R, c, C) else "points"]) for c in (2 * C, C))
+    need = [f.P * (R * 2 // f.th) * c for f, c in ((P2, 2 * C), (P1, C))]
+    if form is not None:
+        need.append((conv0 or F["half" if co.wino_half_applies(R, C, C) else "points"]).P * R * C)
+    return torch.empty(max(need), dtype=torch.float32, device=dev)
 
 
 def require_hip_input(what, x, channels=None):
@@ -379,7 +382,7 @@
                   epilogue=co.EPI_AFFINE_ACT)
 
 
-def _wino_step(geo, x, view, views, wg, wo, V, Mm, h, z, hr, hn, out=None, r=None, cand=None, calls=None):
+def _wino_step(geo, x, view, views, wg, wo, V, Mm, h, z, hr, hn, out=None, r=None, cand=None, calls=None, th=2):
     b, D, H, W = geo
     C = h.shape[-1]
     transform, gemm = calls or co.wino_calls(co.WINO_FORMS["points"])
@@ -387,8 +390,8 @@
     def conv(src, U, Cout, i):
         Vs = transform(src, C, C, b, D, H, W, out=V)
         if isinstance(x, tuple):
-            return Vs, gemm(Vs, C, None, 0, U, Mm, b, D, H // 2, W // 2, Cout), dict(Mm2=x[i], view=view, views=views)
-        return Vs, gemm(x, C, Vs, C, U, Mm, b, D, H // 2, W // 2, Cout, view=view, views=views), {}
+            return Vs, gemm(Vs, C, None, 0, U, Mm, b, D, H // th, W // 2, Cout), dict(Mm2=x[i], view=view, views=views)
+        return Vs, gemm(x, C, Vs, C, U, Mm, b, D, H // th, W // 2, Cout, view=view, views=views), {}
 
     Vh, G, add = conv(h, wg[0], 2 * C, 0)
     co.wino_output(G, wg[1], None, None, 1.0, None, h, None, z, hr, r, *geo, 2 * C, C, co.EPI_GRU_GATES, **add)
@@ -408,8 +411,9 @@
     co.conv_igemm(*ops, *wo, 1.0, res, h, z, hn, out, grid, ig, C, C, taps, epilogue=co.EPI_GRU_OUT, bs1=bs, out3=cand)
 
 
-_WKEY = {None: "_U", co.WINO_FORMS["dn"]: "_Ud", co.WINO_FORMS["dn4"]: "_Ud4"}
-_PACKS = ((None, ("gate", "out", "fc0", "fc3")), (co.WINO_FORMS["dn"], ("gate", "out", "fc0", "fc3")), (co.WINO_FORMS["dn4"], ("gate", "out")))
+_WKEY = {None: "_U", co.WINO_FORMS["dn"]: "_Ud", co.WINO_FORMS["dn4"]: "_Ud4", co.WINO_DN4H: "_Ud4h"}
+_PACKS = ((None, ("gate", "out", "fc0", "fc3")), (co.WINO_FORMS["dn"], ("gate", "out", "fc0", "fc3")), (co.WINO_FORMS["dn4"], ("gate", "out")),
+          (co.WINO_DN4H, ("gate", "out")))
 
 
 def _fuse_eval(gru, xr, groups, wino, split, h0=None, keep=None, const0=None):
@@ -421,9 +425,12 @@
     if wino:
         R = b * D * (H // 2) * (W // 2)
         F = co.WINO_FORMS
-        both = lambda form: all(form.applies(R, D, H // 2, W // 2, c, 2 * C) for c in (2 * C, C))
+        both = lambda form: H % form.th == 0 and all(form.applies(R * 2 // form.th, D, H // form.th, W // 2, c, 2 * C) for c in (2 * C, C))
+        fits = lambda form: co.wino_fits(b, D, H, W, C, views=t, form=form)
         if not split and keep is None and const0 is None and both(F["dn"]):
-            step = F["dn4"] if both(F["dn4"]) and co.wino_fits(b, D, H, W, C, views=t, form=F["dn4"]) else F["dn"]
+            step = F["dn4"] if both(F["dn4"]) and fits(F["dn4"]) else F["dn"]
+            if step is F["dn4"] and both(co.WINO_DN4H) and fits(co.WINO_DN4H):
+                step = co.WINO_DN4H
             conv0 = F["dn"] if F["dn"].applies(R, D, H // 2, W // 2, C, C) else None
     p = gru._packed_halves(wino) if (split or const0 is not None) else gru._packed_wino(step) if wino else gru._packed()
     wk = _WKEY[step] if wino else "_w"
@@ -434,9 +441,9 @@
         X = calls[0](xr, C, C, b * t, D, H, W)
         if split:
             X = (_input_products(X, p["gate_Ux"], b * t, geo, 2 * C), _input_products(X, p["out_Ux"], b * t, geo, C))
-        Vs = torch.empty(16, int(R * (step.rows if step else 1)), C, dtype=torch.float32, device=dev)
+        Vs = torch.empty(step.points, int(R * 2 // step.th * step.rows), C, dtype=torch.float32, device=dev) if step else torch.empty(16, R, C, dtype=torch.float32, device=dev)
         V = Vs.reshape(-1)[:16 * R * C].view(16, R, C)
-        Mm = _step_scratch(R, C, dev, step)
+        Mm = _step_scratch(R, C, dev, step, conv0)
     elif split:
         X = {}
         for ti in sorted({ti for g in groups for ti in g}):
@@ -469,7 +476,7 @@
             elif const0 is not None and k == 0:
                 _wino_step(geo, (const0["MXg0"], const0["MXc0"]), 0, 1, *weights("h"), V, Mm, h, z, hr, hn, last, r, cand)
             else:
-                _wino_step(geo, X, ti, t, wg, wo, Vs, Mm, h, z, hr, hn, last, r, cand, calls=calls)
+                _wino_step(geo, X, ti, t, wg, wo, Vs, Mm, h, z, hr, hn, last, r, cand, calls=calls, th=step.th if step else 2)
             if keep is not None:
                 keep += [h, z, r, cand]
             h, hn = hn, h
@@ -820,6 +827,8 @@
     def _packed_wino(self, form=None):
         p = self._packed()
         for f, convs in _PACKS:
+            if f is not form and convs == ("gate", "out"):
+                continue
             if convs[0] + _WKEY[f] not in p:
                 p.update({k + _WKEY[f]: co.wino_pack(f or co.WINO_FORMS["points"], p[k + "_w"]) for k in convs})
             if f is form:
diff --git a/include/forge_hip.h b/include/forge_hip.h
--- a/include/forge_hip.h
+++ b/include/forge_hip.h
@@ -88,6 +88,13 @@
 int forge_wino_weights_dn4(const float* wp, float* Ud, int Cout, int Cin, forge_stream_t stream);
 int forge_wino_gemm_dn4(const float* V1, int C1, int ld1, long long bs1, long long pt1, const float* V2, int C2, int ld2, long long bs2,
                         long long pt2, const float* Ud, float* Mm, int n, int D, int Ht, int Wt, int Cout, int kd, forge_stream_t stream);
+int forge_wino_input_dn4h(const float* in, int ld, long long bs, float* V, int ldv, long long ptv, int n, int D, int H, int W, int C,
+                          int nsum, long long sum_stride, forge_stream_t stream);
+int forge_wino_weights_dn4h(const float* wp, float* Ud, int Cout, int Cin, forge_stream_t stream);
+int forge_wino_gemm_dn4h(const float* V1, int C1, int ld1, long long bs1, long long pt1, const float* V2, int C2, int ld2, long long bs2,
+                         long long pt2, const float* Ud, float* Mm, int n, int D, int Ht, int Wt, int Cout, int kd, forge_stream_t stream);
+int forge_wino_output_dn4h(const float* Mm, const float* bias, const float* scale, const float* shift, const float* aux_h, const float* aux_z, float* out,
+                           float* out2, float* out3, int n, int D, int H, int W, int Cout, int ldo, int epilogue, forge_stream_t stream);
 int forge_wino_gemm_tile(long long R, int Cout, int Cin);
 int forge_wino_output(const float* Mm, const float* Mm2, long long bs2, long long pt2, const float* bias, const float* scale, const float* shift, float slope, const float* residual,
                       const float* aux_h, const float* aux_z, float* out, float* out2, float* out3, int n, int D, int H, int W, int Cout,
```

After: 1023 views/s, median of 6. +10.2%, better.
